# antoyang/TubeDETR

Measured on AMD Instinct MI355X. Metric: training clips/sec (fwd+bwd) at T=100 k=4 res=352, 1/2/4/8 MI355X, higher is better.
Workload: dtype bf16

## Files before the change

include/tubedetr_hip.h:

```cpp
#ifndef TUBEDETR_HIP_H
#define TUBEDETR_HIP_H
#include <stddef.h>
#include <stdint.h>
#ifdef __cplusplus
extern "C" {
#endif

#define TD_F32 0
#define TD_BF16 1
#define TD_U8 2
#define TD_OK 0
#define TD_ERR_INVALID (-1)
#define TD_ERR_LAUNCH (-2)

typedef void* td_stream_t;

const char* td_last_error(void);
int td_abi_version(void);

int td_set_deterministic(int on);
int td_get_deterministic(void);


#define TD_PROF_GEMM_128x128 0
#define TD_PROF_GEMM_128x64 1
#define TD_PROF_WGRAD 2
#define TD_PROF_GEMM_64x128 3
#define TD_PROF_PW_RESIDENT 4
#define TD_PROF_GEMM_256 5
#define TD_PROF_GEMM_256_PW 6
#define TD_PROF_FUSED 7
#define TD_PROF_CROSS_Q1 8
#define TD_PROF_WGRAD_SINGLE 9
#define TD_PROF_CHAIN 10
#define TD_PROF_FAMILIES 11
int td_prof_enable(int on);
int td_prof_collect(int family, int dtype, long long* launches, double* ms, double* flops);
int td_prof_collect_bytes(int family, int dtype, double* bytes);
int td_prof_dump(const char* path);
int td_debug_set_stamp_buffer(unsigned long long* buf);

typedef struct td_conv_desc {
  int N, Hs, Ws, C;
  int Ho, Wo;
  int R, S, stride, pad;
  int mode;
  int Nc;
  int ldc;
  int out_sp;
  int out_H, out_W;
  int aniso;
  int stride_w, pad_w;
} td_conv_desc;

typedef struct td_epilogue {
  const float* bias;
  const void* residual;
  const void* mask_src;
  int relu;
  int sigmoid;
  float dropout_p;
  uint32_t dropout_seed;
  float alpha;
  const uint32_t* dropout_counter;
} td_epilogue;

int td_conv_gemm(const void* src, const void* wmat, void* out, const td_conv_desc* d, const td_epilogue* e,
                 int dtype, td_stream_t stream);

typedef struct td_linear_ex_desc {
  int M, N, K1, K2;
  int lda1, lda2, ldc, ldr;
  int w_shared;
  long long rows1, rows2;
  const int* a1_map;
  const int* a2_map;
  const int* out_map;
  const int* res_map;
} td_linear_ex_desc;
int td_linear_ex(const void* a1, const void* a2, const void* wmat, void* out, const td_linear_ex_desc* x, const td_epilogue* e,
                 int dtype, td_stream_t stream);

int td_conv_wgrad(const void* g, const void* src, float* dw, const td_conv_desc* d, int ldg, int dtype, int splits,
                  td_stream_t stream);
int td_conv_wgrad_bias(const void* g, const void* src, float* dw, float* dbias, const td_conv_desc* d, int ldg, int dtype,
                       int splits, td_stream_t stream);

typedef struct td_wgrad_job {
  const void* g;
  const void* src;
  float* dW;
  const float* scale;
  td_conv_desc d;
  int ldg;
  int ci_real;
  float* dbias;
  int accumulate;
  int prezeroed;
} td_wgrad_job;
size_t td_conv_wgrad_batch_table_bytes(int n_jobs);
int td_conv_wgrad_batch(const td_wgrad_job* jobs, int n_jobs, int dtype, void* table_host, void* table_dev, size_t table_bytes,
                        td_stream_t stream);

typedef struct td_frame_source {
  const void* data;
  int dtype;
  int n;
  const int* index;
  const int* valid_hw;
} td_frame_source;
int td_frames_to_nhwc(const td_frame_source* srcs, int n_srcs, int C, int H, int W, int Cpad, const float* mean,
                      const float* inv_std, void* y, int dtype, td_stream_t stream);

size_t td_resnet_fwd_ws_bytes(int N, int H, int W, const int* nblocks, int dtype, int save);
int td_resnet_num_convs(const int* nblocks);
int td_resnet_fwd(const td_frame_source* srcs, int n_srcs, const float* mean, const float* inv_std, int N, int H, int W,
                  const int* nblocks, const void* const* w_fwd, const float* const* bias, int save, void* ws, size_t ws_bytes,
                  void** feat, int* feat_hw, int stem_pairs, int first_train_stage, int dtype, td_stream_t stream);
int td_bottleneck_fused(const void* x, void* out, const void* w1, const float* b1, const void* w2, const float* b2, const void* w3,
                        const float* b3, const void* wd, const float* bd, int N, int H, int W, int Cin, int dtype, td_stream_t stream);
int td_pw_chain2(const void* y2, const void* w3, const float* b3, const void* residual, void* out, const void* w1, const float* b1,
                 void* h1, int M, int planes, int dtype, td_stream_t stream);
int td_stem_pair_weights(const void* w_fwd_8, void* w_pairs, int Co, int dtype, td_stream_t stream);
int td_stem_pool(const void* x_pairs, const void* w_pairs, const float* bias, void* pooled, int N, int H, int W, int dtype,
                 td_stream_t stream);
size_t td_resnet_bwd_ws_bytes(int N, int H, int W, const int* nblocks, int first_train_stage, int dtype);
size_t td_resnet_bwd_table_bytes(const int* nblocks, int first_train_stage);
int td_resnet_bwd(const void* dfeat, int N, int N_fwd, int H, int W, const int* nblocks, int first_train_stage,
                  const void* const* w_dgrad, const float* const* scale, float* const* dW, const void* fwd_ws, void* ws,
                  size_t ws_bytes, void* table_host, void* table_dev, size_t table_bytes, int dW_prezeroed, int dtype, int only_stage, td_stream_t stream);

int td_weight_prep(const float* W, const float* bn_w, const float* bn_b, const float* bn_rm, const float* bn_rv,
                   const float* bias, int Co, int Ci, int R, int S, int Cpad, void* w_fwd, void* w_dgrad,
                   float* bias_out, float* scale_out, int dtype, td_stream_t stream);

typedef struct td_prep_item {
  const float* W;
  const float *bn_w, *bn_b, *bn_rm, *bn_rv, *bias;
  void *w_fwd, *w_dgrad;
  float *bias_out, *scale_out;
  int Co, Ci, RS, Cpad, Co_alloc, blk0;
} td_prep_item;
int td_weight_prep_batch(const td_prep_item* items_dev, int n, int total_blocks, int dtype, td_stream_t stream);

int td_wgrad_finalize(const float* dw_k, const float* scale, float* dW, int Co, int Ci, int R, int S, int Cpad,
                      int accumulate, td_stream_t stream);

int td_nchw_to_nhwc(const float* x, void* y, int N, int C, int H, int W, int Cpad, int dtype, td_stream_t stream);
int td_nhwc_to_nchw(const void* x, float* y, int N, int C, int H, int W, int dtype, td_stream_t stream);
int td_cast(const void* x, void* y, size_t n, int src_dtype, int dst_dtype, td_stream_t stream);

int td_maxpool3x3s2(const void* x, void* y, int N, int H, int W, int C, int dtype, td_stream_t stream);

int td_add_layernorm_fwd(const void* x, const void* r, const float* gamma, const float* beta, void* y, void* s_out,
                         float* mean, float* rstd, int rows, int cols, float eps, int dtype, td_stream_t stream);
int td_add_layernorm_bwd(const void* dy, const void* s, const float* mean, const float* rstd, const float* gamma,
                         const void* extra, void* ds, float* dgamma, float* dbeta, int rows, int cols, int dtype,
                         td_stream_t stream);

int td_colsum(const void* g, float* out, int rows, int cols, int ld, int dtype, td_stream_t stream);
int td_add(const void* a, const void* b, void* y, size_t n, int dtype, td_stream_t stream);

int td_relu_bwd(const void* dy, const void* y, void* g, size_t n, float scale, int dtype, td_stream_t stream);

int td_gelu_fwd(const void* x, void* y, size_t n, int dtype, td_stream_t stream);
int td_gelu_bwd(const void* dy, const void* x, void* dx, size_t n, int dtype, td_stream_t stream);

int td_dropout(const void* x, void* y, size_t n, float p, uint32_t seed, const uint32_t* dropout_counter, int dtype,
               td_stream_t stream);

int td_pos_sine(const uint8_t* mask, void* pos, int N, int h, int w, int npf, float temperature, int rows_per_image, int dtype,
                td_stream_t stream);

int td_rows_copy(const void* src, const int* src_map, const void* add, void* dst, const int* dst_map, int n_rows, int cols, int ld_src,
                 int ld_add, int ld_dst, int dtype, td_stream_t stream);
int td_rows_segment_sum(const void* in, const int* idx, const int* ptr, void* out, const int* out_map, int n_out, int cols, int ld_in,
                        int ld_out, int dtype, td_stream_t stream);

int td_mha_fwd(const void* q, const void* k, const void* v, const uint8_t* key_pad, void* out, float* probs,
               float* wavg, int B, int H, int Lq, int Lk, int hd, int ldq, int ldk, int ldv, int ldo, float scale,
               float dropout_p, uint32_t dropout_seed, const uint32_t* dropout_counter, int dtype, td_stream_t stream);
int td_mha_bwd(const void* q, const void* k, const void* v, const void* dout, const float* probs, const float* dwavg,
               void* dq, void* dk, void* dv, float* ds_ws, int B, int H, int Lq, int Lk, int hd, int ldq, int ldk,
               int ldv, int ldo, float scale, float dropout_p, uint32_t dropout_seed, const uint32_t* dropout_counter,
               int dtype, td_stream_t stream);

int td_cross_q1_fwd(const void* u, const void* mem, const void* pos, const uint8_t* key_pad, float* probs, float* wavg, void* zext,
                    int F, int S, int H, int E, int ldz, float dropout_p, uint32_t dropout_seed, const uint32_t* dropout_counter,
                    int dtype, td_stream_t stream);
int td_cross_q1_bwd(const void* u, const void* mem, const void* pos, const float* probs, const void* d_zext, const float* dwavg,
                    void* d_u, float* d_mem, int accumulate, int F, int S, int H, int E, int ldz, float dropout_p, uint32_t dropout_seed,
                    const uint32_t* dropout_counter, int dtype, td_stream_t stream);
int td_cross_q1_bwd_coef(const void* u, const void* mem, const void* pos, const float* probs, const void* d_zext, const float* dwavg,
                         void* d_u, void* coef, int coef_ld, int coef_col, int F, int S, int H, int E, int ldz, float dropout_p,
                         uint32_t dropout_seed, const uint32_t* dropout_counter, int dtype, td_stream_t stream);
int td_cross_q1_dmem(const void* coef, int coef_ld, const void* const* u, const void* const* d_zext, int n_layers, void* d_mem, int F, int S,
                     int H, int E, int ldz, int dtype, td_stream_t stream);
int td_head_blocks_expand(const float* W, const float* bias, float alpha, void* w_n, void* w_t, int E, int H, int dtype, td_stream_t stream);
int td_head_blocks_extract(const float* G, float alpha, float* dW, float* db, int E, int H, td_stream_t stream);

size_t td_mha_lean_stats_bytes(int B, int H, int Lq);
int td_mha_lean_fwd(const void* q, const void* k, const void* v, const uint8_t* key_pad, void* out, float* stats, int B, int H,
                    int Lq, int Lk, int hd, int ldq, int ldk, int ldv, int ldo, float scale, float dropout_p,
                    uint32_t dropout_seed, const uint32_t* dropout_counter, int dtype, td_stream_t stream);
int td_mha_lean_bwd(const void* q, const void* k, const void* v, const uint8_t* key_pad, const void* out, const void* dout,
                    float* stats, void* dq, void* dk, void* dv, int B, int H, int Lq, int Lk, int hd, int ldq, int ldk, int ldv,
                    int ldo, float scale, float dropout_p, uint32_t dropout_seed, const uint32_t* dropout_counter, int dtype,
                    td_stream_t stream);


#define TD_OPTIM_MAX_SEGMENTS 32
// ... 29 lines not shown
```

tubedetr_amd/_hip.py:

```python
from __future__ import annotations

import ctypes as C
import os

import torch

TD_F32, TD_BF16 = 0, 1
EXPECTED_ABI = 10
_LIB_PATH = os.environ.get("TD_HIP_LIB") or os.path.join(os.path.dirname(os.path.abspath(__file__)), "lib", "libtubedetr_hip.so")
_lib = None


class ConvDesc(C.Structure):
    _fields_ = [(n, C.c_int) for n in ("N", "Hs", "Ws", "C", "Ho", "Wo", "R", "S", "stride", "pad", "mode", "Nc", "ldc", "out_sp", "out_H", "out_W",
                                       "aniso", "stride_w", "pad_w")]


class PrepItem(C.Structure):
    _fields_ = [(n, C.c_void_p) for n in ("W", "bn_w", "bn_b", "bn_rm", "bn_rv", "bias", "w_fwd", "w_dgrad", "bias_out", "scale_out")] + \
               [(n, C.c_int) for n in ("Co", "Ci", "RS", "Cpad", "Co_alloc", "blk0")]


class WgradJob(C.Structure):
    _fields_ = [("g", C.c_void_p), ("src", C.c_void_p), ("dW", C.c_void_p), ("scale", C.c_void_p), ("d", ConvDesc), ("ldg", C.c_int), ("ci_real", C.c_int), ("dbias", C.c_void_p), ("accumulate", C.c_int), ("prezeroed", C.c_int)]


TD_U8 = 2


class FrameSource(C.Structure):
    _fields_ = [("data", C.c_void_p), ("dtype", C.c_int), ("n", C.c_int), ("index", C.c_void_p), ("valid_hw", C.c_void_p)]


class LinearExDesc(C.Structure):
    _fields_ = [(n, C.c_int) for n in ("M", "N", "K1", "K2", "lda1", "lda2", "ldc", "ldr", "w_shared")] + \
               [("rows1", C.c_longlong), ("rows2", C.c_longlong)] + [(n, C.c_void_p) for n in ("a1_map", "a2_map", "out_map", "res_map")]


class OptimSegment(C.Structure):
    _fields_ = [("begin", C.c_longlong), ("end", C.c_longlong), ("group", C.c_int), ("active", C.c_int)]


class Epilogue(C.Structure):
    _fields_ = [
        ("bias", C.c_void_p),
        ("residual", C.c_void_p),
        ("mask_src", C.c_void_p),
        ("relu", C.c_int),
        ("sigmoid", C.c_int),
        ("dropout_p", C.c_float),
        ("dropout_seed", C.c_uint32),
        ("alpha", C.c_float),
        ("dropout_counter", C.c_void_p),
    ]


_P, _I, _F, _U32, _SZ = C.c_void_p, C.c_int, C.c_float, C.c_uint32, C.c_size_t
_SIGS = {
    "td_prof_enable": [_I],
    "td_prof_dump": [C.c_char_p],
    "td_debug_set_stamp_buffer": [_P],
    "td_prof_collect": [_I, _I, C.POINTER(C.c_longlong), C.POINTER(C.c_double), C.POINTER(C.c_double)],
    "td_prof_collect_bytes": [_I, _I, C.POINTER(C.c_double)],
    "td_conv_gemm": [_P, _P, _P, C.POINTER(ConvDesc), C.POINTER(Epilogue), _I, _P],
    "td_conv_wgrad": [_P, _P, _P, C.POINTER(ConvDesc), _I, _I, _I, _P],
    "td_conv_wgrad_bias": [_P, _P, _P, _P, C.POINTER(ConvDesc), _I, _I, _I, _P],
    "td_conv_wgrad_batch": [C.POINTER(WgradJob), _I, _I, _P, _P, _SZ, _P],
    "td_resnet_num_convs": [C.POINTER(C.c_int)],
    "td_resnet_fwd": [C.POINTER(FrameSource), _I, C.POINTER(C.c_float), C.POINTER(C.c_float), _I, _I, _I, C.POINTER(C.c_int), C.POINTER(_P), C.POINTER(_P), _I, _P, _SZ,
                      C.POINTER(_P), C.POINTER(C.c_int), _I, _I, _I, _P],
    "td_bottleneck_fused": [_P, _P, _P, _P, _P, _P, _P, _P, _P, _P, _I, _I, _I, _I, _I, _P],
    "td_stem_pair_weights": [_P, _P, _I, _I, _P],
    "td_stem_pool": [_P, _P, _P, _P, _I, _I, _I, _I, _P],
    "td_pw_chain2": [_P, _P, _P, _P, _P, _P, _P, _P, _I, _I, _I, _P],
    "td_set_deterministic": [_I],
    "td_get_deterministic": [],
    "td_frames_to_nhwc": [C.POINTER(FrameSource), _I, _I, _I, _I, _I, C.POINTER(C.c_float), C.POINTER(C.c_float), _P, _I, _P],
    "td_resnet_bwd": [_P, _I, _I, _I, _I, C.POINTER(C.c_int), _I, C.POINTER(_P), C.POINTER(_P), C.POINTER(_P), _P, _P, _SZ, _P, _P, _SZ, _I, _I, _I, _P],
    "td_weight_prep_batch": [_P, _I, _I, _I, _P],
    "td_weight_prep": [_P, _P, _P, _P, _P, _P, _I, _I, _I, _I, _I, _P, _P, _P, _P, _I, _P],
    "td_wgrad_finalize": [_P, _P, _P, _I, _I, _I, _I, _I, _I, _P],
    "td_nchw_to_nhwc": [_P, _P, _I, _I, _I, _I, _I, _I, _P],
    "td_nhwc_to_nchw": [_P, _P, _I, _I, _I, _I, _I, _P],
    "td_cast": [_P, _P, _SZ, _I, _I, _P],
    "td_maxpool3x3s2": [_P, _P, _I, _I, _I, _I, _I, _P],
    "td_add_layernorm_fwd": [_P, _P, _P, _P, _P, _P, _P, _P, _I, _I, _F, _I, _P],
    "td_add_layernorm_bwd": [_P, _P, _P, _P, _P, _P, _P, _P, _P, _I, _I, _I, _P],
    "td_colsum": [_P, _P, _I, _I, _I, _I, _P],
    "td_add": [_P, _P, _P, _SZ, _I, _P],
    "td_relu_bwd": [_P, _P, _P, _SZ, _F, _I, _P],
    "td_gelu_fwd": [_P, _P, _SZ, _I, _P],
    "td_gelu_bwd": [_P, _P, _P, _SZ, _I, _P],
    "td_dropout": [_P, _P, _SZ, _F, _U32, _P, _I, _P],
    "td_pos_sine": [_P, _P, _I, _I, _I, _I, _F, _I, _I, _P],
    "td_linear_ex": [_P, _P, _P, _P, C.POINTER(LinearExDesc), C.POINTER(Epilogue), _I, _P],
    "td_rows_copy": [_P, _P, _P, _P, _P, _I, _I, _I, _I, _I, _I, _P],
    "td_rows_segment_sum": [_P, _P, _P, _P, _P, _I, _I, _I, _I, _I, _P],
    "td_criterion_fwd": [_P, _P, _P, _P, _P, _P, _P, _P, _P, _F, _F, _I, _I, _I, _I, _P, _P, _P, _P, _P, _P],
    "td_criterion_bwd": [_P, _P, _P, _P, _P, _P, _P, _P, _I, _I, _I, _P],
    "td_sted_decode": [_P, _P, _I, _I, _P],
    "td_grad_norm_clip": [_P, _SZ, C.POINTER(OptimSegment), _I, _F, _P, _SZ, _P, _P, _P],
    "td_adamw_ema_step": [_P, _P, _P, _P, _P, _SZ, C.POINTER(OptimSegment), _I, _P, _P, _P, _F, _F, _F, _F, _F, _P],
    "td_mha_fwd": [_P, _P, _P, _P, _P, _P, _P, _I, _I, _I, _I, _I, _I, _I, _I, _I, _F, _F, _U32, _P, _I, _P],
    "td_mha_bwd": [_P, _P, _P, _P, _P, _P, _P, _P, _P, _P, _I, _I, _I, _I, _I, _I, _I, _I, _I, _F, _F, _U32, _P, _I, _P],
    "td_cross_q1_fwd": [_P, _P, _P, _P, _P, _P, _P, _I, _I, _I, _I, _I, _F, _U32, _P, _I, _P],
    "td_cross_q1_bwd": [_P, _P, _P, _P, _P, _P, _P, _P, _I, _I, _I, _I, _I, _I, _F, _U32, _P, _I, _P],
    "td_cross_q1_bwd_coef": [_P, _P, _P, _P, _P, _P, _P, _P, _I, _I, _I, _I, _I, _I, _I, _F, _U32, _P, _I, _P],
    "td_cross_q1_dmem": [_P, _I, _P, _P, _I, _P, _I, _I, _I, _I, _I, _I, _P],
    "td_head_blocks_expand": [_P, _P, _F, _P, _P, _I, _I, _I, _P],
    "td_head_blocks_extract": [_P, _F, _P, _P, _I, _I, _P],
    "td_mha_lean_fwd": [_P, _P, _P, _P, _P, _P, _I, _I, _I, _I, _I, _I, _I, _I, _I, _F, _F, _U32, _P, _I, _P],
    "td_mha_lean_bwd": [_P, _P, _P, _P, _P, _P, _P, _P, _P, _P, _I, _I, _I, _I, _I, _I, _I, _I, _I, _F, _F, _U32, _P, _I, _P],
}
_SIZE_SIGS = {
    "td_grad_norm_ws_bytes": [],
    "td_mha_lean_stats_bytes": [_I, _I, _I],
    "td_conv_wgrad_batch_table_bytes": [_I],
    "td_resnet_bwd_table_bytes": [C.POINTER(C.c_int), _I],
    "td_resnet_fwd_ws_bytes": [_I, _I, _I, C.POINTER(C.c_int), _I, _I],
    "td_resnet_bwd_ws_bytes": [_I, _I, _I, C.POINTER(C.c_int), _I, _I],
}
EXPORTS = ["td_last_error", "td_abi_version"] + list(_SIGS) + list(_SIZE_SIGS)


def lib_path() -> str:
    return _LIB_PATH


def lib() -> C.CDLL:
    global _lib
    if _lib is None:
        if not os.path.exists(_LIB_PATH):
            raise RuntimeError(
                f"{_LIB_PATH} is missing: build it with `python -m tubedetr_amd.build` (or __graft_entry__.build()); "
                "tubedetr_amd has no CPU / eager fallback"
            )
        L = C.CDLL(_LIB_PATH)
        L.td_last_error.restype = C.c_char_p
        L.td_last_error.argtypes = []
        L.td_abi_version.restype = C.c_int
# ... 40 lines not shown
```

tubedetr_amd/csrc/api.cpp:

```cpp
#include <stdarg.h>

#include <atomic>
#include <mutex>
#include <vector>

#include "td_common.h"

namespace td {

static thread_local char g_err[512] = "";

void set_error(const char* fmt, ...) {
  va_list ap;
  va_start(ap, fmt);
  vsnprintf(g_err, sizeof(g_err), fmt, ap);
  va_end(ap);
}

int check_launch(const char* what) {
  hipError_t e = hipGetLastError();
  if (e != hipSuccess) {
    set_error("%s: launch failed: %s", what, hipGetErrorString(e));
    return TD_ERR_LAUNCH;
  }
// ... 49 lines not shown
}
extern "C" int td_get_deterministic(void) { return td::deterministic() ? 1 : 0; }

extern "C" int td_prof_enable(int on) {
  std::lock_guard<std::mutex> lk(td::g_prof_mu);
  td::g_prof.store(on != 0);
  if (on) {
    for (auto& r : td::g_recs) { td::g_pool.push_back(r.a); td::g_pool.push_back(r.b); }
    td::g_recs.clear();
  }
  return TD_OK;
}
extern "C" int td_prof_collect(int family, int dtype, long long* launches, double* ms, double* flops) {
  long long n = 0; double t = 0, f = 0;
  std::lock_guard<std::mutex> lk(td::g_prof_mu);
  for (auto& r : td::g_recs) {
    if (r.family != family || r.dtype != dtype) continue;
    if (hipEventSynchronize(r.b) != hipSuccess) { td::set_error("td_prof_collect: event sync failed"); return TD_ERR_LAUNCH; }
    float e = 0.f;
    hipEventElapsedTime(&e, r.a, r.b);
    n++; t += e; f += r.flops;
  }
  if (launches) *launches = n;
  if (ms) *ms = t;
  if (flops) *flops = f;
  return TD_OK;
}

extern "C" int td_prof_collect_bytes(int family, int dtype, double* bytes) {
  double b = 0;
  std::lock_guard<std::mutex> lk(td::g_prof_mu);
  for (auto& r : td::g_recs)
    if (r.family == family && r.dtype == dtype) b += r.bytes;
  if (bytes) *bytes = b;
  return TD_OK;
}

extern "C" int td_prof_dump(const char* path) {
  FILE* f = fopen(path, "w");
  if (!f) { td::set_error("td_prof_dump: cannot open %s", path); return TD_ERR_INVALID; }
  fprintf(f, "family,dtype,M,N,K,R,stride,mode,ms\n");
  std::lock_guard<std::mutex> lk(td::g_prof_mu);
  for (auto& r : td::g_recs) {
    hipEventSynchronize(r.b);
    float e = 0.f;
    hipEventElapsedTime(&e, r.a, r.b);
    fprintf(f, "%d,%d,%d,%d,%d,%d,%d,%d,%.5f\n", r.family, r.dtype, r.M, r.N, r.K, r.R, r.stride, r.mode, e);
  }
  fclose(f);
  return TD_OK;
}

extern "C" const char* td_last_error(void) { return td::g_err; }
extern "C" int td_abi_version(void) { return 10; }
```

tubedetr_amd/csrc/elementwise.hip:

```cpp
#include "td_common.h"

namespace td {

template <typename T>
__global__ void maxpool3x3s2_kernel(const T* x, T* y, int N, int H, int W, int C, int Ho, int Wo) {
  constexpr int VEC = 16 / sizeof(T);
  const int cv = C / VEC;
  const size_t n = (size_t)N * Ho * Wo * cv;
  const size_t idx = (size_t)blockIdx.x * blockDim.x + threadIdx.x;
  if (idx >= n) return;
  int c = (idx % cv) * VEC;
  size_t t = idx / cv;
  int wo = t % Wo; t /= Wo;
  int ho = t % Ho;
  int img = t / Ho;
  float m[VEC];
#pragma unroll
  for (int i = 0; i < VEC; ++i) m[i] = -INFINITY;
  for (int r = 0; r < 3; ++r) {
    int h = ho * 2 - 1 + r;
    if ((unsigned)h >= (unsigned)H) continue;
    for (int s = 0; s < 3; ++s) {
      int w = wo * 2 - 1 + s;
      if ((unsigned)w >= (unsigned)W) continue;
// ... 69 lines not shown
}
static bool aligned8(const void* a, const void* b, const void* c, const void* d) {
  return (((uintptr_t)a | (uintptr_t)b | (uintptr_t)c | (uintptr_t)d) & 7) == 0;
}

template <int NJ>
__global__ __launch_bounds__(256) void add_layernorm_fwd_v4_kernel(const u16* __restrict__ x, const u16* __restrict__ r, const float* __restrict__ gamma,
                                                                   const float* __restrict__ beta, u16* __restrict__ y, u16* __restrict__ s_out,
                                                                   float* __restrict__ mean, float* __restrict__ rstd, int rows, float eps) {
  constexpr int cols = NJ * 256;
  const int lane = threadIdx.x & 63;
  const int row = blockIdx.x * 4 + (threadIdx.x >> 6);
  if (row >= rows) return;
  const size_t base = (size_t)row * cols + lane * 4;
  float v[NJ][4];
  float sum = 0.f;
#pragma unroll
  for (int j = 0; j < NJ; ++j) {
    unpack4v(*(const uint2*)(x + base + 256 * j), v[j]);
    if (r) {
      float a[4];
      unpack4v(*(const uint2*)(r + base + 256 * j), a);
#pragma unroll
      for (int e = 0; e < 4; ++e) v[j][e] += a[e];
    }
#pragma unroll
    for (int e = 0; e < 4; ++e) sum += v[j][e];
  }
  const float mu = wave_sum(sum) * (1.f / cols);
  float var = 0.f;
#pragma unroll
  for (int j = 0; j < NJ; ++j)
#pragma unroll
    for (int e = 0; e < 4; ++e) {
      const float d = v[j][e] - mu;
      var += d * d;
    }
  var = wave_sum(var) * (1.f / cols);
  const float rs = rsqrtf(var + eps);
  if (lane == 0) {
    if (mean) mean[row] = mu;
    if (rstd) rstd[row] = rs;
  }
#pragma unroll
  for (int j = 0; j < NJ; ++j) {
    const float4 gm = *(const float4*)(gamma + lane * 4 + 256 * j), bt = *(const float4*)(beta + lane * 4 + 256 * j);
    if (s_out) *(uint2*)(s_out + base + 256 * j) = pack4_bf16(v[j]);
    float o[4] = {(v[j][0] - mu) * rs * gm.x + bt.x, (v[j][1] - mu) * rs * gm.y + bt.y, (v[j][2] - mu) * rs * gm.z + bt.z,
                  (v[j][3] - mu) * rs * gm.w + bt.w};
    *(uint2*)(y + base + 256 * j) = pack4_bf16(o);
  }
}

template <int NJ>
__global__ __launch_bounds__(256) void add_layernorm_bwd_v4_kernel(const u16* __restrict__ dy, const u16* __restrict__ s, const float* __restrict__ mean,
                                                                   const float* __restrict__ rstd, const float* __restrict__ gamma,
                                                                   const u16* __restrict__ extra, u16* __restrict__ ds, float* dgamma, float* dbeta,
                                                                   int rows) {
  constexpr int cols = NJ * 256;
  const int lane = threadIdx.x & 63;
  const int wid = blockIdx.x * 4 + (threadIdx.x >> 6);
  const int nw = gridDim.x * 4;
  float pg[NJ][4], pb[NJ][4], gm[NJ][4];
#pragma unroll
  for (int j = 0; j < NJ; ++j) {
    const float4 g4 = *(const float4*)(gamma + lane * 4 + 256 * j);
    gm[j][0] = g4.x; gm[j][1] = g4.y; gm[j][2] = g4.z; gm[j][3] = g4.w;
#pragma unroll
    for (int e = 0; e < 4; ++e) pg[j][e] = pb[j][e] = 0.f;
  }
  for (int row = wid; row < rows; row += nw) {
    const size_t base = (size_t)row * cols + lane * 4;
    const float mu = mean[row], rs = rstd[row];
    float xh[NJ][4], dg[NJ][4];
    float c1 = 0.f, c2 = 0.f;
#pragma unroll
    for (int j = 0; j < NJ; ++j) {
      float d[4], sv[4];
      unpack4v(*(const uint2*)(dy + base + 256 * j), d);
      unpack4v(*(const uint2*)(s + base + 256 * j), sv);
#pragma unroll
      for (int e = 0; e < 4; ++e) {
        xh[j][e] = (sv[e] - mu) * rs;
        dg[j][e] = d[e] * gm[j][e];
        c1 += dg[j][e];
        c2 += dg[j][e] * xh[j][e];
        pg[j][e] += d[e] * xh[j][e];
        pb[j][e] += d[e];
      }
    }
    c1 = wave_sum(c1) * (1.f / cols);
    c2 = wave_sum(c2) * (1.f / cols);
#pragma unroll
    for (int j = 0; j < NJ; ++j) {
      float o[4];
#pragma unroll
      for (int e = 0; e < 4; ++e) o[e] = rs * (dg[j][e] - c1 - xh[j][e] * c2);
      if (extra) {
        float ex[4];
        unpack4v(*(const uint2*)(extra + base + 256 * j), ex);
#pragma unroll
        for (int e = 0; e < 4; ++e) o[e] += ex[e];
      }
      *(uint2*)(ds + base + 256 * j) = pack4_bf16(o);
    }
  }
  __shared__ float redg[4][cols], redb[4][cols];
  const int wv = threadIdx.x >> 6;
#pragma unroll
  for (int j = 0; j < NJ; ++j)
#pragma unroll
    for (int e = 0; e < 4; ++e) {
      redg[wv][lane * 4 + 256 * j + e] = pg[j][e];
      redb[wv][lane * 4 + 256 * j + e] = pb[j][e];
    }
  __syncthreads();
  for (int c = threadIdx.x; c < cols; c += 256) {
    if (dgamma) atomicAdd(dgamma + c, redg[0][c] + redg[1][c] + redg[2][c] + redg[3][c]);
    if (dbeta) atomicAdd(dbeta + c, redb[0][c] + redb[1][c] + redb[2][c] + redb[3][c]);
  }
}

template <typename T>
__global__ __launch_bounds__(256) void add_layernorm_bwd_kernel(const T* dy, const T* s, const float* mean, const float* rstd,
                                                                const float* gamma, const T* extra, T* ds, float* dgamma,
                                                                float* dbeta, int rows, int cols) {
  const int lane = threadIdx.x & 63;
  const int wid = blockIdx.x * 4 + (threadIdx.x >> 6);
  const int nw = gridDim.x * 4;
  const int nj = (cols + 63) / 64;
  float pg[LN_MAXJ], pb[LN_MAXJ];
#pragma unroll
  for (int j = 0; j < LN_MAXJ; ++j) pg[j] = pb[j] = 0.f;
  for (int row = wid; row < rows; row += nw) {
    const size_t base = (size_t)row * cols;
    const float mu = mean[row], rs = rstd[row];
    float xh[LN_MAXJ], dg[LN_MAXJ];
    float c1 = 0.f, c2 = 0.f;
#pragma unroll
    for (int j = 0; j < LN_MAXJ; ++j) {
      xh[j] = dg[j] = 0.f;
      int c = lane + 64 * j;
      if (j < nj && c < cols) {
        float d = Elem<T>::load(dy, base + c);
        xh[j] = (Elem<T>::load(s, base + c) - mu) * rs;
        dg[j] = d * gamma[c];
        c1 += dg[j];
        c2 += dg[j] * xh[j];
        pg[j] += d * xh[j];
        pb[j] += d;
      }
    }
    c1 = wave_sum(c1) / cols;
    c2 = wave_sum(c2) / cols;
#pragma unroll
    for (int j = 0; j < LN_MAXJ; ++j) {
      int c = lane + 64 * j;
      if (j < nj && c < cols) {
        float o = rs * (dg[j] - c1 - xh[j] * c2);
        if (extra) o += Elem<T>::load(extra, base + c);
        Elem<T>::store(ds, base + c, o);
      }
    }
  }
  __shared__ float redg[4][64 * LN_MAXJ], redb[4][64 * LN_MAXJ];
  const int wv = threadIdx.x >> 6;
#pragma unroll
  for (int j = 0; j < LN_MAXJ; ++j) {
    if (j < nj) {
      redg[wv][lane + 64 * j] = pg[j];
      redb[wv][lane + 64 * j] = pb[j];
    }
  }
  __syncthreads();
  for (int c = threadIdx.x; c < cols; c += 256) {
    if (dgamma) atomicAdd(dgamma + c, redg[0][c] + redg[1][c] + redg[2][c] + redg[3][c]);
    if (dbeta) atomicAdd(dbeta + c, redb[0][c] + redb[1][c] + redb[2][c] + redb[3][c]);
  }
}

template <typename T>
__global__ void colsum_kernel(const T* g, float* out, int rows, int cols, int ld, int rows_per_block) {
  const int c = blockIdx.x * blockDim.x + threadIdx.x;
  if (c >= cols) return;
  const int r0 = blockIdx.y * rows_per_block;
  const int r1 = min(rows, r0 + rows_per_block);
  float acc = 0.f;
  for (int r = r0; r < r1; ++r) acc += Elem<T>::load(g, (size_t)r * ld + c);
  atomicAdd(out + c, acc);
}

template <typename T>
__global__ __launch_bounds__(256) void colsum_vec_kernel(const T* g, float* out, int rows, int cols, int ld, int rows_per_block) {
  constexpr int VEC = 16 / sizeof(T);
  __shared__ float red[8][32 * VEC + 1];
  const int cg = threadIdx.x & 31, rl = threadIdx.x >> 5;
  const int c0 = (blockIdx.x * 32 + cg) * VEC;
  const int r0 = blockIdx.y * rows_per_block;
  const int r1 = min(rows, r0 + rows_per_block);
  float acc[VEC];
#pragma unroll
  for (int i = 0; i < VEC; ++i) acc[i] = 0.f;
  if (c0 < cols) {
    for (int r = r0 + rl; r < r1; r += 8) {
      uint4 v = *(const uint4*)(g + (size_t)r * ld + c0);
      const T* e = (const T*)&v;
#pragma unroll
      for (int i = 0; i < VEC; ++i) acc[i] += Elem<T>::load(e, i);
    }
  }
#pragma unroll
  for (int i = 0; i < VEC; ++i) red[rl][cg * VEC + i] = acc[i];
  __syncthreads();
  for (int c = threadIdx.x; c < 32 * VEC; c += 256) {
// ... 192 lines not shown
  size_t n = (size_t)N * Ho * Wo * (C / vec);
  hipStream_t st = (hipStream_t)stream;
  TD_DISPATCH(dtype, (maxpool3x3s2_kernel<u16><<<nblk(n), 256, 0, st>>>((const u16*)x, (u16*)y, N, H, W, C, Ho, Wo)),
              (maxpool3x3s2_kernel<float><<<nblk(n), 256, 0, st>>>((const float*)x, (float*)y, N, H, W, C, Ho, Wo)),
              "td_maxpool3x3s2");
  return check_launch("td_maxpool3x3s2");
}

extern "C" int td_add_layernorm_fwd(const void* x, const void* r, const float* gamma, const float* beta, void* y,
                                    void* s_out, float* mean, float* rstd, int rows, int cols, float eps, int dtype,
                                    td_stream_t stream) {
  TD_REQUIRE(x && gamma && beta && y, "td_add_layernorm_fwd: null pointer");
  TD_REQUIRE(cols <= 64 * LN_MAXJ, "td_add_layernorm_fwd: cols > %d", 64 * LN_MAXJ);
  if (rows == 0) return TD_OK;
  hipStream_t st = (hipStream_t)stream;
  unsigned g = (rows + 3) / 4;
  if (dtype == TD_BF16 && (cols == 256 || cols == 768) && aligned8(x, r, y, s_out)) {
    if (cols == 256) add_layernorm_fwd_v4_kernel<1><<<g, 256, 0, st>>>((const u16*)x, (const u16*)r, gamma, beta, (u16*)y, (u16*)s_out, mean, rstd, rows, eps);
    else add_layernorm_fwd_v4_kernel<3><<<g, 256, 0, st>>>((const u16*)x, (const u16*)r, gamma, beta, (u16*)y, (u16*)s_out, mean, rstd, rows, eps);
    return check_launch("td_add_layernorm_fwd");
  }
  TD_DISPATCH(dtype,
              (add_layernorm_fwd_kernel<u16><<<g, 256, 0, st>>>((const u16*)x, (const u16*)r, gamma, beta, (u16*)y, (u16*)s_out, mean, rstd, rows, cols, eps)),
              (add_layernorm_fwd_kernel<float><<<g, 256, 0, st>>>((const float*)x, (const float*)r, gamma, beta, (float*)y, (float*)s_out, mean, rstd, rows, cols, eps)),
              "td_add_layernorm_fwd");
  return check_launch("td_add_layernorm_fwd");
}

extern "C" int td_add_layernorm_bwd(const void* dy, const void* s, const float* mean, const float* rstd,
                                    const float* gamma, const void* extra, void* ds, float* dgamma, float* dbeta,
                                    int rows, int cols, int dtype, td_stream_t stream) {
  TD_REQUIRE(dy && s && mean && rstd && gamma && ds, "td_add_layernorm_bwd: null pointer");
  TD_REQUIRE(cols <= 64 * LN_MAXJ, "td_add_layernorm_bwd: cols > %d", 64 * LN_MAXJ);
  if (rows == 0) return TD_OK;
  hipStream_t st = (hipStream_t)stream;
  unsigned g = (rows + 3) / 4;
  if (dtype == TD_BF16 && (cols == 256 || cols == 768) && aligned8(dy, s, ds, extra)) {
    unsigned gv = (rows + 31) / 32;
    if (gv > 1024) gv = 1024;
    if (deterministic()) gv = 1;
    if (cols == 256) add_layernorm_bwd_v4_kernel<1><<<gv, 256, 0, st>>>((const u16*)dy, (const u16*)s, mean, rstd, gamma, (const u16*)extra, (u16*)ds, dgamma, dbeta, rows);
    else add_layernorm_bwd_v4_kernel<3><<<gv, 256, 0, st>>>((const u16*)dy, (const u16*)s, mean, rstd, gamma, (const u16*)extra, (u16*)ds, dgamma, dbeta, rows);
    return check_launch("td_add_layernorm_bwd");
  }
  if (g > 256) g = 256;
  if (deterministic()) g = 1;
  TD_DISPATCH(dtype,
              (add_layernorm_bwd_kernel<u16><<<g, 256, 0, st>>>((const u16*)dy, (const u16*)s, mean, rstd, gamma, (const u16*)extra, (u16*)ds, dgamma, dbeta, rows, cols)),
              (add_layernorm_bwd_kernel<float><<<g, 256, 0, st>>>((const float*)dy, (const float*)s, mean, rstd, gamma, (const float*)extra, (float*)ds, dgamma, dbeta, rows, cols)),
              "td_add_layernorm_bwd");
  return check_launch("td_add_layernorm_bwd");
}

extern "C" int td_colsum(const void* g, float* out, int rows, int cols, int ld, int dtype, td_stream_t stream) {
  TD_REQUIRE(g && out, "td_colsum: null pointer");
  if (rows == 0 || cols == 0) return TD_OK;
  hipStream_t st = (hipStream_t)stream;
  const int vec = dtype == TD_BF16 ? 8 : 4;
  if (cols % vec == 0 && ld % vec == 0) {
    const int gx = (cols + 32 * vec - 1) / (32 * vec);
    int rpb = (int)(((long long)rows * gx + 511) / 512);
    if (rpb < 64) rpb = 64;
    if (deterministic()) rpb = rows;
    dim3 grid(gx, (rows + rpb - 1) / rpb);
    TD_DISPATCH(dtype, (colsum_vec_kernel<u16><<<grid, 256, 0, st>>>((const u16*)g, out, rows, cols, ld, rpb)),
                (colsum_vec_kernel<float><<<grid, 256, 0, st>>>((const float*)g, out, rows, cols, ld, rpb)), "td_colsum");
    return check_launch("td_colsum");
  }
  int rpb = (int)(((long long)rows * ((cols + 255) / 256) + 1023) / 1024);
  if (rpb < 8) rpb = 8;
  if (deterministic()) rpb = rows;
  dim3 grid((cols + 255) / 256, (rows + rpb - 1) / rpb);
  TD_DISPATCH(dtype, (colsum_kernel<u16><<<grid, 256, 0, st>>>((const u16*)g, out, rows, cols, ld, rpb)),
              (colsum_kernel<float><<<grid, 256, 0, st>>>((const float*)g, out, rows, cols, ld, rpb)), "td_colsum");
  return check_launch("td_colsum");
}

extern "C" int td_add(const void* a, const void* b, void* y, size_t n, int dtype, td_stream_t stream) {
  TD_REQUIRE(a && y, "td_add: null pointer");
  if (n == 0) return TD_OK;
  hipStream_t st = (hipStream_t)stream;
  unsigned g = nblk(n / 4 + 1);
  if (g > 4096) g = 4096;
  TD_REQUIRE(((uintptr_t)a | (uintptr_t)y | (uintptr_t)b) % 16 == 0, "td_add: pointers must be 16-byte aligned");
  TD_DISPATCH(dtype, (ew_kernel<u16, 0><<<g, 256, 0, st>>>((const u16*)a, (const u16*)b, (u16*)y, n, 1.f, 0, 0, nullptr)),
              (ew_kernel<float, 0><<<g, 256, 0, st>>>((const float*)a, (const float*)b, (float*)y, n, 1.f, 0, 0, nullptr)), "td_add");
  return check_launch("td_add");
}

extern "C" int td_relu_bwd(const void* dy, const void* y, void* g, size_t n, float scale, int dtype, td_stream_t stream) {
  TD_REQUIRE(dy && y && g, "td_relu_bwd: null pointer");
  if (n == 0) return TD_OK;
  hipStream_t st = (hipStream_t)stream;
  unsigned gr = nblk(n);
  if (gr > 4096) gr = 4096;
  TD_REQUIRE(((uintptr_t)dy | (uintptr_t)y | (uintptr_t)g) % 16 == 0, "td_relu_bwd: pointers must be 16-byte aligned");
  TD_DISPATCH(dtype, (ew_kernel<u16, 1><<<gr, 256, 0, st>>>((const u16*)dy, (const u16*)y, (u16*)g, n, scale, 0, 0, nullptr)),
              (ew_kernel<float, 1><<<gr, 256, 0, st>>>((const float*)dy, (const float*)y, (float*)g, n, scale, 0, 0, nullptr)), "td_relu_bwd");
  return check_launch("td_relu_bwd");
}

extern "C" int td_gelu_fwd(const void* x, void* y, size_t n, int dtype, td_stream_t stream) {
  TD_REQUIRE(x && y, "td_gelu_fwd: null pointer");
  if (n == 0) return TD_OK;
  hipStream_t st = (hipStream_t)stream;
  unsigned gr = nblk(n);
// ... 87 lines not shown
```

tubedetr_amd/csrc/gemm_conv.hip:

```cpp
#include <stdlib.h>

#include <type_traits>

#include "td_common.h"
#include <algorithm>
#include <vector>

#ifndef TD_WGRAD_EARLY_ISSUE
#define TD_WGRAD_EARLY_ISSUE 1
#endif
#ifndef TD_BIG_XCD_CONTIG
#define TD_BIG_XCD_CONTIG 1
#endif
namespace td {

struct GemmParams {
  const char* src;
  const char* w;
  char* out;
  td_conv_desc d;
  int M, K;
  uint32_t src_bytes, w_bytes;
  unsigned long long* dbg;
  const float* bias;
  const char* residual;
  const char* mask_src;
  int relu, sigmoid;
  float alpha;
  uint32_t drop_thresh;
  float drop_scale;
  uint32_t seed;
  const uint32_t* seed_dev;
  const char* src2;
  uint32_t src2_bytes;
  int K1, lda1, lda2, ldr;
  int w_shared;
  const int* a1_map;
  const int* a2_map;
  const int* out_map;
  const int* res_map;
  int tap_inner;
  int w_ld;
  int wtap[4];
  int use_wtap;
};

template <typename T>
struct Mfma;
template <>
struct Mfma<u16> {
  static __device__ __forceinline__ void run(const uint4& wf, const uint4& af, f32x4& acc) {
    acc = __builtin_amdgcn_mfma_f32_16x16x32_bf16(*(const bf16x8*)&wf, *(const bf16x8*)&af, acc, 0, 0, 0);
  }
};
template <>
struct Mfma<float> {
  static __device__ __forceinline__ void run(const uint4& wf, const uint4& af, f32x4& acc) {
    const float* a = (const float*)&wf;
    const float* b = (const float*)&af;
#pragma unroll
    for (int s = 0; s < 4; ++s) acc = __builtin_amdgcn_mfma_f32_16x16x4f32(a[s], b[s], acc, 0, 0, 0);
  }
};

template <typename T>
__device__ __forceinline__ void load4(const char* base, size_t off, float (&o)[4]);
template <>
__device__ __forceinline__ void load4<float>(const char* base, size_t off, float (&o)[4]) {
  float4 v = *(const float4*)(base + off * 4);
  o[0] = v.x; o[1] = v.y; o[2] = v.z; o[3] = v.w;
}
template <>
__device__ __forceinline__ void load4<u16>(const char* base, size_t off, float (&o)[4]) {
  uint2 v = *(const uint2*)(base + off * 2);
  o[0] = __uint_as_float(v.x << 16); o[1] = __uint_as_float(v.x & 0xffff0000u);
  o[2] = __uint_as_float(v.y << 16); o[3] = __uint_as_float(v.y & 0xffff0000u);
}
template <typename T, typename V>
__device__ __forceinline__ void unpack4(const V& v, float (&o)[4]);
template <>
__device__ __forceinline__ void unpack4<float, float4>(const float4& v, float (&o)[4]) {
  o[0] = v.x; o[1] = v.y; o[2] = v.z; o[3] = v.w;
}
template <>
__device__ __forceinline__ void unpack4<u16, uint2>(const uint2& v, float (&o)[4]) {
  o[0] = __uint_as_float(v.x << 16); o[1] = __uint_as_float(v.x & 0xffff0000u);
  o[2] = __uint_as_float(v.y << 16); o[3] = __uint_as_float(v.y & 0xffff0000u);
}
typedef __bf16 bf16x2_t __attribute__((ext_vector_type(2)));
__device__ __forceinline__ uint32_t pack_bf16x2(float lo, float hi) {
  bf16x2_t v = {(__bf16)lo, (__bf16)hi};
  return *(uint32_t*)&v;
}
template <typename T>
__device__ __forceinline__ void unpack16(const uint4& v, float (&o)[16 / sizeof(T)]);
template <>
__device__ __forceinline__ void unpack16<float>(const uint4& v, float (&o)[4]) {
  o[0] = __uint_as_float(v.x); o[1] = __uint_as_float(v.y); o[2] = __uint_as_float(v.z); o[3] = __uint_as_float(v.w);
}
template <>
__device__ __forceinline__ void unpack16<u16>(const uint4& v, float (&o)[8]) {
  o[0] = __uint_as_float(v.x << 16); o[1] = __uint_as_float(v.x & 0xffff0000u);
  o[2] = __uint_as_float(v.y << 16); o[3] = __uint_as_float(v.y & 0xffff0000u);
  o[4] = __uint_as_float(v.z << 16); o[5] = __uint_as_float(v.z & 0xffff0000u);
  o[6] = __uint_as_float(v.w << 16); o[7] = __uint_as_float(v.w & 0xffff0000u);
}
template <typename T>
__device__ __forceinline__ uint4 pack16(const float (&v)[16 / sizeof(T)]);
template <>
__device__ __forceinline__ uint4 pack16<float>(const float (&v)[4]) {
  return make_uint4(__float_as_uint(v[0]), __float_as_uint(v[1]), __float_as_uint(v[2]), __float_as_uint(v[3]));
}
template <>
__device__ __forceinline__ uint4 pack16<u16>(const float (&v)[8]) {
  return make_uint4(pack_bf16x2(v[0], v[1]), pack_bf16x2(v[2], v[3]), pack_bf16x2(v[4], v[5]), pack_bf16x2(v[6], v[7]));
}
template <typename T>
__device__ __forceinline__ void store4(char* base, size_t off, const float (&v)[4]);
template <>
__device__ __forceinline__ void store4<float>(char* base, size_t off, const float (&v)[4]) {
  *(float4*)(base + off * 4) = make_float4(v[0], v[1], v[2], v[3]);
}
template <>
__device__ __forceinline__ void store4<u16>(char* base, size_t off, const float (&v)[4]) {
  uint2 o;
  o.x = (uint32_t)f32_to_bf16(v[0]) | ((uint32_t)f32_to_bf16(v[1]) << 16);
  o.y = (uint32_t)f32_to_bf16(v[2]) | ((uint32_t)f32_to_bf16(v[3]) << 16);
  *(uint2*)(base + off * 2) = o;
}

__device__ __forceinline__ float sigmoidf_(float x) { return 1.f / (1.f + __expf(-x)); }

typedef __attribute__((address_space(3))) void* lds_ptr_t;

#ifndef TD_NT
#define TD_NT 3
#endif
typedef uint32_t u32x4_t __attribute__((ext_vector_type(4)));
typedef uint32_t u32x2_t __attribute__((ext_vector_type(2)));
__device__ __forceinline__ uint4 ld16(const char* p) {
#if TD_NT & 1
  const u32x4_t v = __builtin_nontemporal_load((const u32x4_t*)p);
  return make_uint4(v.x, v.y, v.z, v.w);
#else
  return *(const uint4*)p;
#endif
// ... 272 lines not shown
  issue_tile(nxt);                                                                  \
  if ((j) >= 0) compute_tile(cur);
    for (int it = -2; it < nk; it += 3) {
      TD_CG_STEP(smem1, smem0, it)
      if (it + 1 >= nk) break;
      TD_CG_STEP(smem2, smem1, it + 1)
      if (it + 2 >= nk) break;
      TD_CG_STEP(smem0, smem2, it + 2)
    }
#undef TD_CG_STEP
    asm volatile("s_waitcnt vmcnt(0)" ::: "memory");
    TD_STAMP(2);
    fetch_epilogue_operands();
  }

  asm volatile("s_waitcnt lgkmcnt(0)" ::: "memory");
  __builtin_amdgcn_s_barrier();
  TD_STAMP(3);
  float* stg = (float*)((wave < 2 ? smem0 : smem1) + (wave & 1) * (WM * WN * 4));
  const float alpha = p.alpha;
#pragma unroll
  for (int j = 0; j < TM; ++j) {
    const int row = j * 16 + lr;
#pragma unroll
    for (int i = 0; i < TN; ++i) {
      const int c = (i * 4 + lg) ^ (row & (CPRW - 1));
      f32x4 a = acc[i][j];
      *(float4*)(stg + row * WN + c * 4) = make_float4(a[0] * alpha, a[1] * alpha, a[2] * alpha, a[3] * alpha);
    }
  }
  asm volatile("s_waitcnt lgkmcnt(0)" ::: "memory");
  float bias[EPL];
#pragma unroll
  for (int r = 0; r < EPL; ++r) bias[r] = (p.bias && n + r < d.Nc) ? p.bias[n + r] : 0.f;
  TD_STAMP(4);
  const uint32_t eff_seed = effective_seed(p.seed, p.drop_thresh ? p.seed_dev : nullptr);
#pragma unroll
  for (int it = 0; it < NIT; ++it) {
    if (!live[it]) continue;
    const int row = it * RPI + rsub;
    const int sw = row & (CPRW - 1);
    float v[EPL];
#pragma unroll
    for (int q = 0; q < EPL / 4; ++q) {
      float4 f = *(const float4*)(stg + row * WN + (((cc * (EPL / 4) + q) ^ sw) * 4));
      v[4 * q + 0] = f.x + bias[4 * q + 0]; v[4 * q + 1] = f.y + bias[4 * q + 1];
      v[4 * q + 2] = f.z + bias[4 * q + 2]; v[4 * q + 3] = f.w + bias[4 * q + 3];
    }
    const size_t off = offs[it];
    if (vec_ok) {
      if (p.residual) {
        float r8[EPL];
        unpack16<T>(res[it], r8);
#pragma unroll
        for (int r = 0; r < EPL; ++r) v[r] += r8[r];
      }
      if (p.relu) {
#pragma unroll
        for (int r = 0; r < EPL; ++r) v[r] = fmaxf(v[r], 0.f);
      }
      if (p.sigmoid) {
#pragma unroll
        for (int r = 0; r < EPL; ++r) v[r] = sigmoidf_(v[r]);
      }
      if (p.mask_src) {
        float m8[EPL];
        unpack16<T>(msk[it], m8);
#pragma unroll
        for (int r = 0; r < EPL; ++r) v[r] = m8[r] > 0.f ? v[r] : 0.f;
      }
      if (p.drop_thresh) {
#pragma unroll
        for (int r = 0; r < EPL; ++r) v[r] = dropout_keep(eff_seed, (uint32_t)(off + r), p.drop_thresh) ? v[r] * p.drop_scale : 0.f;
      }
      st16(p.out + off * ES, pack16<T>(v));
    } else {
      const int cnt = min(EPL, d.Nc - n);
      for (int r = 0; r < cnt; ++r) {
        float x = v[r];
        if (p.residual) x += Elem<T>::load(p.residual, (GX ? roffs[it] : off) + r);
        if (p.relu) x = fmaxf(x, 0.f);
        if (p.sigmoid) x = sigmoidf_(x);
        if (p.mask_src) x = Elem<T>::load(p.mask_src, off + r) > 0.f ? x : 0.f;
        if (p.drop_thresh) x = dropout_keep(eff_seed, (uint32_t)(off + r), p.drop_thresh) ? x * p.drop_scale : 0.f;
        Elem<T>::store(p.out, off + r, x);
      }
    }
  }
  TD_STAMP(5);
#undef TD_STAMP
}

#ifndef TD_ABL
#define TD_ABL 0
#endif
template <int OFF>
__device__ __forceinline__ u32x4_t lds_read16(uint32_t addr) {
  u32x4_t r;
#if TD_ABL & 4
  asm volatile("" : "=v"(r) : "v"(addr));
#else
  asm volatile("ds_read_b128 %0, %1 offset:%2" : "=v"(r) : "v"(addr), "n"(OFF));
#endif
  return r;
}
template <int N>
__device__ __forceinline__ void wait_vmcnt() {
  asm volatile("s_waitcnt vmcnt(%0)" ::"n"(N) : "memory");
}
template <int I>
using ic = std::integral_constant<int, I>;

#ifndef TD_BIG8_AUX_W
#define TD_BIG8_AUX_W 0
#endif
#ifndef TD_BIG8_AUX_X
#define TD_BIG8_AUX_X 0
#endif
template <bool TU, bool RES>
__global__ __launch_bounds__(512, 1) void conv_gemm_big8_kernel(GemmParams p) {
  using T = u16;
  constexpr int ES = 2, BM = 256, BN = 256, BK = 64, NW = 8, VEC = 8;
  constexpr int WM = 128, WN = 64, TM = 8, TN = 4;
  constexpr int STAGE = (BM + BN) * 128, WREG = BM * 128;
  constexpr uint32_t OOB = 0xFFFFFFF0u;
  constexpr int MAXT = 160;
  constexpr int STG = 16 * WN * ES;
  __shared__ __attribute__((aligned(16))) char smem[2 * STAGE];
  __shared__ __attribute__((aligned(16))) uint4 ktab[MAXT];
  __shared__ __attribute__((aligned(16))) char stg_all[NW * STG];

  const td_conv_desc& d = p.d;
  const int t = threadIdx.x;
// ... 201 lines not shown
      for (int j = 0; j < TM; ++j) acc[i][j] = f32x4{0.f, 0.f, 0.f, 0.f};
    taddr = tab0 + 2 * 16;
    f32x4 bs[TN];
#pragma unroll
    for (int i = 0; i < TN; ++i) bs[i] = p.bias ? *(const f32x4*)(p.bias + n0 + wx * WN + i * 16 + lg * 4) : f32x4{0.f, 0.f, 0.f, 0.f};
    wait_vmcnt<7>();
    __builtin_amdgcn_s_barrier();
    if (wy == 1) __builtin_amdgcn_s_barrier();
    TD_STAMP(1);
    const int npair = (nk + 1) / 2;
#pragma unroll 1
    for (int it = 0; it < npair; ++it) {
      phase(ic<0>{}, ic<0>{}); phase(ic<0>{}, ic<1>{}); phase(ic<0>{}, ic<2>{}); phase(ic<0>{}, ic<3>{});
      phase(ic<1>{}, ic<0>{}); phase(ic<1>{}, ic<1>{}); phase(ic<1>{}, ic<2>{}); phase(ic<1>{}, ic<3>{});
    }
    if (wy == 0) __builtin_amdgcn_s_barrier();
    TD_STAMP(2);
    asm volatile("s_waitcnt vmcnt(0) lgkmcnt(0)" ::: "memory");
    asm volatile("s_nop 15\n\ts_nop 15" ::: "memory");
#pragma unroll
    for (int i = 0; i < TN; ++i)
#pragma unroll
      for (int j = 0; j < TM; ++j) asm volatile("" : "+v"(acc[i][j]));
#pragma unroll
    for (int i = 0; i < TN; ++i) asm volatile("" : "+v"(bs[i]));
    const int vb_next = vb + (int)gridDim.x;
    const bool more = tile_ok(vb_next);
    if (more) {
      tile_addr(tile_m0(vb_next), tile_n0(vb_next));
      prologue_issue();
    }
    TD_STAMP(3);
    uint4 mk[2][2];
    auto seg_off = [&](int j, int h) -> uint32_t {
      const int m = m0 + wy * WM + j * 16 + h * 8 + rsub;
      return m < p.M ? ((uint32_t)m * (uint32_t)d.ldc + (uint32_t)(n0 + wx * WN + cc * 8)) * ES : OOB;
    };
    auto fetch_mask = [&](int j, int b) {
#pragma unroll
      for (int h = 0; h < 2; ++h) {
        const uint32_t off = seg_off(j, h);
        mk[b][h] = off != OOB ? ld16(p.mask_src + off) : make_uint4(0, 0, 0, 0);
      }
    };
    auto put = [&](int j) {
#pragma unroll
      for (int i = 0; i < TN; ++i) {
        const f32x4 a = acc[i][j];
        float v[4] = {a[0] * alpha + bs[i][0], a[1] * alpha + bs[i][1], a[2] * alpha + bs[i][2], a[3] * alpha + bs[i][3]};
        if constexpr (RES) {
          const int m = m0 + wy * WM + j * 16 + lr;
          if (m < p.M) {
            const uint2 rr = *(const uint2*)(p.residual + ((size_t)m * d.ldc + n0 + wx * WN + i * 16 + lg * 4) * ES);
            v[0] += __uint_as_float(rr.x << 16); v[1] += __uint_as_float(rr.x & 0xffff0000u);
            v[2] += __uint_as_float(rr.y << 16); v[3] += __uint_as_float(rr.y & 0xffff0000u);
          }
        }
        if (p.relu) {
#pragma unroll
          for (int r = 0; r < 4; ++r) v[r] = fmaxf(v[r], 0.f);
        }
        const uint32_t lo = pack_bf16x2(v[0], v[1]), hi = pack_bf16x2(v[2], v[3]);
        asm volatile("ds_write_b64 %0, %1" ::"v"(swa[i]), "v"(u32x2_t{lo, hi}) : "memory");
      }
    };
    if (p.mask_src) fetch_mask(0, 0);
    put(0);
    u32x4_t o0, o1;
    asm volatile("ds_read_b128 %0, %1" : "=v"(o0) : "v"(sra) : "memory");
    asm volatile("ds_read_b128 %0, %1 offset:1024" : "=v"(o1) : "v"(sra) : "memory");
#pragma unroll
    for (int j = 0; j < TM; ++j) {
      const int b = j & 1;
      if (j + 1 < TM) {
        if (p.mask_src) fetch_mask(j + 1, b ^ 1);
        put(j + 1);
        asm volatile("s_waitcnt lgkmcnt(4)" : "+v"(o0), "+v"(o1) : : "memory");
      } else {
        asm volatile("s_waitcnt lgkmcnt(0)" : "+v"(o0), "+v"(o1) : : "memory");
      }
      u32x4_t s0 = o0, s1 = o1;
      if (j + 1 < TM) {
        asm volatile("ds_read_b128 %0, %1" : "=v"(o0) : "v"(sra) : "memory");
        asm volatile("ds_read_b128 %0, %1 offset:1024" : "=v"(o1) : "v"(sra) : "memory");
      }
      if (p.mask_src) {
        float x8[8], m8[8];
        unpack16<T>(make_uint4(s0.x, s0.y, s0.z, s0.w), x8);
        unpack16<T>(mk[b][0], m8);
#pragma unroll
        for (int r = 0; r < 8; ++r) x8[r] = m8[r] > 0.f ? x8[r] : 0.f;
        const uint4 q0 = pack16<T>(x8);
        s0 = u32x4_t{q0.x, q0.y, q0.z, q0.w};
        unpack16<T>(make_uint4(s1.x, s1.y, s1.z, s1.w), x8);
        unpack16<T>(mk[b][1], m8);
#pragma unroll
        for (int r = 0; r < 8; ++r) x8[r] = m8[r] > 0.f ? x8[r] : 0.f;
        const uint4 q1 = pack16<T>(x8);
        s1 = u32x4_t{q1.x, q1.y, q1.z, q1.w};
      }
      __builtin_amdgcn_raw_buffer_store_b128(s0, rs_out, (int)seg_off(j, 0), 0, 0);
      __builtin_amdgcn_raw_buffer_store_b128(s1, rs_out, (int)seg_off(j, 1), 0, 0);
    }
    TD_STAMP(5);
    if (p.dbg && t == 0) p.dbg[(size_t)vb * 8 + 7] = wall_clock64();
    if (!more) break;
// ... 191 lines not shown
  if (grp == 1) __builtin_amdgcn_s_barrier();
  TD_STAMP(1);
  const int ntri = (nk + 2) / 3;
#pragma unroll 1
  for (int it = 0; it < ntri; ++it) {
    phase(ic<0>{}, ic<0>{}); phase(ic<0>{}, ic<1>{});
    phase(ic<1>{}, ic<0>{}); phase(ic<1>{}, ic<1>{});
    phase(ic<2>{}, ic<0>{}); phase(ic<2>{}, ic<1>{});
  }
  if (grp == 0) __builtin_amdgcn_s_barrier();
  TD_STAMP(2);
  asm volatile("s_waitcnt vmcnt(0) lgkmcnt(0)" ::: "memory");
  asm volatile("s_nop 15\n\ts_nop 15" ::: "memory");
#pragma unroll
  for (int i = 0; i < TN; ++i)
#pragma unroll
    for (int j = 0; j < TM; ++j) asm volatile("" : "+v"(acc[i][j]));
  fetch_chunk(0, 0);
  __builtin_amdgcn_s_barrier();
  TD_STAMP(3);
  float* stg = (float*)(smem + wave * (CR * WN * 4));
  const float alpha = p.alpha;
  float bias[EPL];
#pragma unroll
  for (int r = 0; r < EPL; ++r) bias[r] = p.bias ? p.bias[n + r] : 0.f;
#pragma unroll
  for (int c = 0; c < NCH; ++c) {
    const int b = c & 1;
    {
      const int row = lr;
#pragma unroll
      for (int i = 0; i < TN; ++i) {
        const int cx = (i * 4 + lg) ^ (row & (CPRW - 1));
        const f32x4 a = acc[i][c];
        *(float4*)(stg + row * WN + cx * 4) = make_float4(a[0] * alpha, a[1] * alpha, a[2] * alpha, a[3] * alpha);
      }
    }
    if (c + 1 < NCH) fetch_chunk(c + 1, b ^ 1);
    asm volatile("s_waitcnt lgkmcnt(0)" ::: "memory");
#pragma unroll
    for (int it = 0; it < NIT; ++it) {
      const int row = it * RPI + rsub;
      const int sw = row & (CPRW - 1);
      float v[EPL];
#pragma unroll
      for (int q = 0; q < EPL / 4; ++q) {
        const float4 f = *(const float4*)(stg + row * WN + (((cc * (EPL / 4) + q) ^ sw) * 4));
        v[4 * q + 0] = f.x + bias[4 * q + 0]; v[4 * q + 1] = f.y + bias[4 * q + 1];
        v[4 * q + 2] = f.z + bias[4 * q + 2]; v[4 * q + 3] = f.w + bias[4 * q + 3];
      }
      if (p.residual) {
        float r8[EPL];
        unpack16<T>(res[b][it], r8);
#pragma unroll
        for (int r = 0; r < EPL; ++r) v[r] += r8[r];
      }
      if (p.relu) {
#pragma unroll
        for (int r = 0; r < EPL; ++r) v[r] = fmaxf(v[r], 0.f);
      }
      if (p.mask_src) {
        float m8[EPL];
        unpack16<T>(msk[b][it], m8);
#pragma unroll
        for (int r = 0; r < EPL; ++r) v[r] = m8[r] > 0.f ? v[r] : 0.f;
      }
      if (live[b][it]) st16(p.out + offs[b][it] * ES, pack16<T>(v));
    }
    asm volatile("s_waitcnt lgkmcnt(0)" ::: "memory");
  }
  TD_STAMP(5);
#undef TD_STAMP
}

template <int NKT, bool RES, bool MSK>
__global__ __launch_bounds__(256, 2) void pw_resident2_kernel(GemmParams p, int MT, int P) {
  using T = u16;
  constexpr int ES = 2;
  constexpr uint32_t OOB = 0xFFFFFFF0u;
  constexpr int WM = 32, WN = 64, TM = 2, TN = 4;
  constexpr int CPRW = WN / 4, EPL = 8, LPR = WN / EPL, RPI = 64 / LPR, NIT = WM / RPI;
  constexpr int NOPS = NIT * ((RES ? 1 : 0) + (MSK ? 1 : 0));
  constexpr bool AHEAD = NOPS > 0 && !(RES && MSK && NKT == 4);
  constexpr int NA = 2 * NKT;
  constexpr int AUX_NT = (TD_NT & 2) ? 2 : 0;
  __shared__ __attribute__((aligned(16))) char sA0[32768];
  __shared__ __attribute__((aligned(16))) char sA1[32768];
  __shared__ __attribute__((aligned(16))) char sT[4 * 16 * WN * 4];
  const td_conv_desc& d = p.d;
  const int t = threadIdx.x;
  const int wave = __builtin_amdgcn_readfirstlane(t >> 6), lane = t & 63;
  const int NT = d.Nc >> 7;
  const int xcd = blockIdx.x & 7, local = blockIdx.x >> 3;
  const int GPX = P / NT;
  const int nt = local % NT, gl = local / NT;
  if (gl >= GPX) return;
  const int gid = xcd * GPX + gl, G = 8 * GPX;
  const int lrow = lane >> 3, chunk = (lane & 7) ^ lrow;
  const uint32_t out_bytes = (uint32_t)p.M * (uint32_t)d.ldc * ES;
  const __amdgpu_buffer_rsrc_t rs_src = __builtin_amdgcn_make_buffer_rsrc((void*)p.src, 0, p.src_bytes, 0x00020000);
  const __amdgpu_buffer_rsrc_t rs_out = __builtin_amdgcn_make_buffer_rsrc((void*)p.out, 0, out_bytes, 0x00020000);
  const __amdgpu_buffer_rsrc_t rs_res = __builtin_amdgcn_make_buffer_rsrc((void*)(RES ? p.residual : p.out), 0, out_bytes, 0x00020000);
  const __amdgpu_buffer_rsrc_t rs_msk = __builtin_amdgcn_make_buffer_rsrc((void*)(MSK ? p.mask_src : p.out), 0, out_bytes, 0x00020000);
  const int n0 = nt * 128;
  const int HoWo = d.Ho * d.Wo;
  const bool strided = d.stride != 1;
// ... 61 lines not shown
    for (int i = 0; i < TN; ++i)
#pragma unroll
      for (int j = 0; j < TM; ++j) acc[i][j] = f32x4{0.f, 0.f, 0.f, 0.f};
#pragma unroll
    for (int kt = 0; kt < NKT; ++kt)
#pragma unroll
      for (int ks = 0; ks < 2; ++ks) {
        const int cidx = ks * 4 + lg;
        uint4 af[TM];
#pragma unroll
        for (int j = 0; j < TM; ++j) {
          const int row = wy * WM + j * 16 + lr;
          af[j] = *(const uint4*)(cur + kt * 8192 + row * 128 + ((cidx ^ (row & 7)) << 4));
        }
#pragma unroll
        for (int i = 0; i < TN; ++i)
#pragma unroll
          for (int j = 0; j < TM; ++j) Mfma<T>::run(wfr[kt][ks][i], af[j], acc[i][j]);
      }
    asm volatile("s_waitcnt lgkmcnt(0)" ::: "memory");
    __builtin_amdgcn_s_barrier();
    issue_A(cur, mt + 2 * G);
    if constexpr (AHEAD) fetch_ops(mt + G, B ^ 1);
    if constexpr (NOPS > 0) {
      wait_vmcnt<NA + (AHEAD ? NOPS : 0)>();
      __builtin_amdgcn_sched_barrier(0);
    }
    constexpr int RB = AHEAD ? B : 0;
#pragma unroll
    for (int j = 0; j < TM; ++j) {
#pragma unroll
      for (int i = 0; i < TN; ++i) {
        const int c = (i * 4 + lg) ^ (lr & (CPRW - 1));
        const f32x4 a = acc[i][j];
        *(float4*)(stg + lr * WN + c * 4) = make_float4(a[0], a[1], a[2], a[3]);
      }
      asm volatile("s_waitcnt lgkmcnt(0)" ::: "memory");
#pragma unroll
      for (int h = 0; h < 16 / RPI; ++h) {
        const int it = j * (16 / RPI) + h;
        const int row = h * RPI + rsub;
        const int sw = row & (CPRW - 1);
        float v[EPL];
#pragma unroll
        for (int q = 0; q < EPL / 4; ++q) {
          const float4 f = *(const float4*)(stg + row * WN + (((cc * (EPL / 4) + q) ^ sw) * 4));
          v[4 * q + 0] = f.x + bias[4 * q + 0]; v[4 * q + 1] = f.y + bias[4 * q + 1];
          v[4 * q + 2] = f.z + bias[4 * q + 2]; v[4 * q + 3] = f.w + bias[4 * q + 3];
        }
        const uint32_t off = seg_off(mt, it);
        if constexpr (RES) {
          float r8[EPL];
          unpack16<T>(make_uint4(res[RB][it].x, res[RB][it].y, res[RB][it].z, res[RB][it].w), r8);
#pragma unroll
          for (int r = 0; r < EPL; ++r) v[r] += r8[r];
        }
        if (p.relu) {
#pragma unroll
          for (int r = 0; r < EPL; ++r) v[r] = fmaxf(v[r], 0.f);
        }
        if constexpr (MSK) {
          float m8[EPL];
          unpack16<T>(make_uint4(msk[RB][it].x, msk[RB][it].y, msk[RB][it].z, msk[RB][it].w), m8);
#pragma unroll
          for (int r = 0; r < EPL; ++r) v[r] = m8[r] > 0.f ? v[r] : 0.f;
        }
        if (p.drop_thresh) {
#pragma unroll
          for (int r = 0; r < EPL; ++r) v[r] = dropout_keep(drop_seed, off / ES + (uint32_t)r, p.drop_thresh) ? v[r] * p.drop_scale : 0.f;
        }
        const uint4 o = pack16<T>(v);
        __builtin_amdgcn_raw_buffer_store_b128(u32x4_t{o.x, o.y, o.z, o.w}, rs_out, (int)off, 0, AUX_NT);
      }
      asm volatile("s_waitcnt lgkmcnt(0)" ::: "memory");
    }
  };

  int mt = gid;
  issue_A(sA0, mt);
  issue_A(sA1, mt + G);
  if constexpr (AHEAD) fetch_ops(mt, 0);
  while (mt < MT) {
    step(sA0, sA1, mt, ic<0>{});
    mt += G;
    if (mt >= MT) break;
    step(sA1, sA0, mt, ic<1>{});
    mt += G;
  }
  asm volatile("s_waitcnt vmcnt(0)" ::: "memory");
}

struct WgradParams {
  const char* g;
  const char* src;
  float* dw;
  const float* scale;
  float* dbias;
  td_conv_desc d;
  int M, K, ldg, mper;
  uint32_t g_bytes, src_bytes;
  int out_mode;
  int ci_real;
  int tn, tk, first;
  int cls;
  unsigned long long* stamps;
};
// ... 800 lines not shown
      }
      sub.w_bytes = wbytes - (size_t)(wp - (const char*)w_dgrad);
      const int rc = conv_gemm_launch(g, wp, (char*)dx + ooff, &c, &ec, dtype, stream, &sub);
      if (rc) return rc;
    }
  return TD_OK;
}

extern "C" int td_conv_gemm(const void* src, const void* wmat, void* out, const td_conv_desc* d, const td_epilogue* e,
                            int dtype, td_stream_t stream) {
  TD_REQUIRE(src && wmat && out && d, "td_conv_gemm: null pointer");
  static const int parity = [] { const char* e_ = getenv("TD_DGRAD_S2_PARITY"); return e_ ? atoi(e_) : 1; }();
  if (parity && dtype == TD_BF16 && d->mode == 1 && d->stride == 2 && d->R == 3 && d->S == 3 && d->pad == 1 && !d->aniso && d->out_sp <= 1 &&
      d->Ho == 2 * d->Hs && d->Wo == 2 * d->Ws && d->C % 64 == 0 && d->ldc >= d->Nc && !(e && (e->dropout_p > 0.f || e->sigmoid))) {
    int rc = validate(d, dtype, "td_conv_gemm");
    if (rc) return rc;
    return conv_dgrad_s2_by_parity(src, wmat, out, d, e, dtype, stream);
  }
  return conv_gemm_launch(src, wmat, out, d, e, dtype, stream, nullptr);
}

static int conv_gemm_launch(const void* src, const void* wmat, void* out, const td_conv_desc* d, const td_epilogue* e, int dtype,
                            td_stream_t stream, const WeightSubset* sub) {
  TD_REQUIRE(src && wmat && out && d, "td_conv_gemm: null pointer");
  int rc = validate(d, dtype, "td_conv_gemm");
  if (rc) return rc;
  GemmParams p;
  memset(&p, 0, sizeof(p));
  p.src = (const char*)src;
  p.w = (const char*)wmat;
  p.out = (char*)out;
  p.d = *d;
  if (p.d.out_sp < 1) p.d.out_sp = 1;
  p.M = d->N * d->Ho * d->Wo;
  p.K = d->R * d->S * d->C;
  {
    const double es = dtype == TD_BF16 ? 2.0 : 4.0;
    const double sb = (double)d->N * d->Hs * d->Ws * d->C * es, wb = (double)d->Nc * p.K * es;
    TD_REQUIRE(sb < 4294967000.0 && wb < 4294967000.0, "td_conv_gemm: operand exceeds the 4 GiB buffer-descriptor range");
    p.src_bytes = (uint32_t)sb;
    p.w_bytes = (uint32_t)wb;
  }
  if (sub) {
    p.w_ld = sub->w_ld;
    p.w_bytes = (uint32_t)sub->w_bytes;
    p.use_wtap = sub->ntap > 1;
    for (int i = 0; i < 4; ++i) p.wtap[i] = sub->wtap[i];
  }
  p.alpha = 1.f;
  p.dbg = g_dbg;
  if (e) {
    p.bias = e->bias;
    p.residual = (const char*)e->residual;
    p.mask_src = (const char*)e->mask_src;
    p.relu = e->relu;
    p.sigmoid = e->sigmoid;
    if (e->alpha != 0.f) p.alpha = e->alpha;
    if (e->dropout_p > 0.f) {
      TD_REQUIRE(e->dropout_p < 1.f, "td_conv_gemm: dropout_p must be < 1");
      p.drop_thresh = (uint32_t)((double)e->dropout_p * 4294967296.0);
      if (p.drop_thresh == 0) p.drop_thresh = 1;
      p.drop_scale = 1.f / (1.f - e->dropout_p);
      p.seed = e->dropout_seed;
      p.seed_dev = e->dropout_counter;
    }
  }
  TD_REQUIRE(d->ldc >= d->Nc, "td_conv_gemm: ldc < Nc");
  hipStream_t st = (hipStream_t)stream;
  static const int n_cu = [] {
    int dev = 0, cus = 256;
    if (hipGetDevice(&dev) == hipSuccess) (void)hipDeviceGetAttribute(&cus, hipDeviceAttributeMultiprocessorCount, dev);
    return cus;
  }();
  {
    static const int persist = [] { const char* e_ = getenv("TD_PW_PERSIST"); return e_ ? atoi(e_) : 1; }();
    static const int persist_dropout = [] { const char* e_ = getenv("TD_PW_PERSIST_DROPOUT"); return e_ ? atoi(e_) : 1; }();
    const bool pw0 = d->R == 1 && d->S == 1 && d->pad == 0 && p.d.out_sp == 1 && !d->aniso &&
                     ((d->stride == 1 && d->Hs == d->Ho && d->Ws == d->Wo) ||
                      (d->stride > 1 && d->mode == 0 && (d->Ho - 1) * d->stride < d->Hs && (d->Wo - 1) * d->stride < d->Ws));
    const int NTp = d->Nc / 128, Pp = 2 * n_cu / 8;
    const bool shape_ok = pw0 && !p.w_ld && dtype == TD_BF16 && p.K % 64 == 0 && p.K <= 256 && d->Nc % 128 == 0 &&
                          (NTp == 1 || NTp == 2 || NTp == 4 || NTp == 8 || NTp == 16) && Pp >= NTp && d->ldc % 8 == 0 && !p.sigmoid &&
                          p.alpha == 1.f && n_cu % 8 == 0 && (!p.drop_thresh || persist_dropout) && (double)p.M * d->ldc < 2147483000.0;
    const int MTp = cdiv(p.M, 64);
    const int groups = shape_ok ? 8 * (Pp / NTp) : 1;
    if (persist && shape_ok && MTp >= persist_min_tiles() * groups && !(persist == 2 && p.mask_src) && !(persist == 3 && d->mode != 0)) {
      const bool prof_ = prof_on();
      if (prof_) {
        prof_begin(TD_PROF_PW_RESIDENT, dtype, 2.0 * p.M * d->Nc * p.K, st, p.M, d->Nc, p.K, d->R, d->stride, d->mode);
        const double es_ = 2.0;
        double by = ((double)p.M * p.K + (double)d->Nc * p.K + (double)p.M * d->Nc) * es_;
        if (p.residual) by += (double)p.M * d->Nc * es_;
        if (p.mask_src) by += (double)p.M * d->Nc * es_;
        prof_set_bytes(by);
      }
      const int nkt = p.K / 64;
      const bool hr = p.residual != nullptr, hm = p.mask_src != nullptr;
      dim3 g2(2 * n_cu);
#define TD_PWR(NK)                                                                               \
  do {                                                                                           \
    if (hr && hm) pw_resident2_kernel<NK, true, true><<<g2, 256, 0, st>>>(p, MTp, Pp);          \
    else if (hr) pw_resident2_kernel<NK, true, false><<<g2, 256, 0, st>>>(p, MTp, Pp);          \
    else if (hm) pw_resident2_kernel<NK, false, true><<<g2, 256, 0, st>>>(p, MTp, Pp);          \
    else pw_resident2_kernel<NK, false, false><<<g2, 256, 0, st>>>(p, MTp, Pp);                 \
  } while (0)
      if (nkt == 1) TD_PWR(1);
// ... 81 lines not shown
    else TD_LAUNCH(float, 128, 128);
  }
#undef TD_LAUNCH
  if (prof) prof_end(st);
  return check_launch("td_conv_gemm");
}

extern "C" int td_linear_ex(const void* a1, const void* a2, const void* wmat, void* out, const td_linear_ex_desc* x, const td_epilogue* e,
                            int dtype, td_stream_t stream) {
  TD_REQUIRE(a1 && wmat && out && x, "td_linear_ex: null pointer");
  TD_REQUIRE(dtype == TD_F32 || dtype == TD_BF16, "td_linear_ex: bad dtype %d", dtype);
  const int vec = dtype == TD_BF16 ? 8 : 4, bk = dtype == TD_BF16 ? 64 : 32;
  const int es = dtype == TD_BF16 ? 2 : 4;
  const int K2 = a2 ? x->K2 : 0;
  TD_REQUIRE(x->M >= 1 && x->N >= 1 && x->K1 >= vec && K2 >= 0, "td_linear_ex: bad sizes");
  TD_REQUIRE(x->K1 % vec == 0 && K2 % vec == 0 && x->lda1 % vec == 0 && (!a2 || x->lda2 % vec == 0), "td_linear_ex: K1 / K2 / lda must be multiples of %d", vec);
  TD_REQUIRE(!a2 || x->K1 % bk == 0, "td_linear_ex: with a second source K1=%d must be a multiple of the K tile (%d)", x->K1, bk);
  TD_REQUIRE(x->lda1 >= x->K1 && (!a2 || x->lda2 >= K2) && x->ldc >= x->N, "td_linear_ex: row stride smaller than the row");
  TD_REQUIRE(x->rows1 >= 1 && (!a2 || x->rows2 >= 1) && (x->a1_map || x->rows1 >= x->M) && (!a2 || x->a2_map || x->rows2 >= x->M),
             "td_linear_ex: source has fewer rows than M and no row map");
  GemmParams p;
  memset(&p, 0, sizeof(p));
  p.src = (const char*)a1;
  p.src2 = (const char*)a2;
  p.w = (const char*)wmat;
  p.out = (char*)out;
  p.M = x->M;
  p.K = x->K1 + K2;
  p.K1 = x->K1;
  p.lda1 = x->lda1;
  p.lda2 = a2 ? x->lda2 : 0;
  p.ldr = x->ldr > 0 ? x->ldr : x->ldc;
  p.w_shared = (a2 && x->w_shared) ? 1 : 0;
  TD_REQUIRE(!p.w_shared || K2 == x->K1, "td_linear_ex: a shared weight needs K2 == K1");
  p.a1_map = x->a1_map;
  p.a2_map = a2 ? x->a2_map : nullptr;
  p.out_map = x->out_map;
  p.res_map = x->res_map;
  td_conv_desc d;
  memset(&d, 0, sizeof(d));
  d.N = 1; d.Hs = x->M; d.Ws = 1; d.C = p.K; d.Ho = x->M; d.Wo = 1; d.R = d.S = 1; d.stride = 1; d.Nc = x->N; d.ldc = x->ldc; d.out_sp = 1;
  p.d = d;
  {
    const double b1 = (double)x->rows1 * x->lda1 * es, b2 = a2 ? (double)x->rows2 * x->lda2 * es : 16.0, wb = (double)x->N * (p.w_shared ? x->K1 : p.K) * es;
    TD_REQUIRE(b1 < 4294967000.0 && b2 < 4294967000.0 && wb < 4294967000.0, "td_linear_ex: operand exceeds the 4 GiB buffer-descriptor range");
    p.src_bytes = (uint32_t)b1;
    p.src2_bytes = (uint32_t)b2;
    p.w_bytes = (uint32_t)wb;
  }
  p.alpha = 1.f;
  if (e) {
    p.bias = e->bias;
    p.residual = (const char*)e->residual;
    p.mask_src = (const char*)e->mask_src;
    p.relu = e->relu;
    p.sigmoid = e->sigmoid;
    if (e->alpha != 0.f) p.alpha = e->alpha;
    if (e->dropout_p > 0.f) {
      TD_REQUIRE(e->dropout_p < 1.f, "td_linear_ex: dropout_p must be < 1");
      p.drop_thresh = (uint32_t)((double)e->dropout_p * 4294967296.0);
      if (p.drop_thresh == 0) p.drop_thresh = 1;
      p.drop_scale = 1.f / (1.f - e->dropout_p);
      p.seed = e->dropout_seed;
      p.seed_dev = e->dropout_counter;
    }
  }
  hipStream_t st = (hipStream_t)stream;
  const bool narrow = x->N <= 64;
  const int tiles128 = cdiv(p.M, 128) * cdiv(x->N, 128);
  const bool small_m = !narrow && (tiles128 < 512 || p.K <= 512);
  const int BMsel = small_m ? 64 : 128, BNsel = narrow ? 64 : 128;
  dim3 grid(8 * cdiv(cdiv(p.M, BMsel), 8) * cdiv(x->N, BNsel));
  const bool prof = prof_on();
  if (prof) {
    prof_begin(narrow ? TD_PROF_GEMM_128x64 : (small_m ? TD_PROF_GEMM_64x128 : TD_PROF_GEMM_128x128), dtype, 2.0 * p.M * x->N * p.K, st, p.M, x->N, p.K, 1, 1, 2);
    double by = ((double)p.M * p.K + (double)x->N * p.K + (double)p.M * x->N) * es;
    if (p.residual) by += (double)p.M * x->N * es;
    if (p.mask_src) by += (double)p.M * x->N * es;
    prof_set_bytes(by);
  }
#define TD_LX(TT)                                                                                     \
  do {                                                                                                \
    if (narrow) conv_gemm_kernel<TT, 128, 64, 2, true, false, true><<<grid, 256, 0, st>>>(p);         \
    else if (small_m) conv_gemm_kernel<TT, 64, 128, 2, true, false, true><<<grid, 256, 0, st>>>(p);   \
    else conv_gemm_kernel<TT, 128, 128, 2, true, false, true><<<grid, 256, 0, st>>>(p);               \
  } while (0)
  if (dtype == TD_BF16) TD_LX(u16);
  else TD_LX(float);
#undef TD_LX
  if (prof) prof_end(st);
  return check_launch("td_linear_ex");
}

static int wgrad_stages() {
  static const int nstg = [] { const char* e = getenv("TD_WGRAD_STAGES"); return (e && atoi(e) == 2) ? 2 : 4; }();
  return nstg;
}

static int wgrad_fill(WgradParams& p, const void* g, const void* src, const td_conv_desc* d, int ldg, int dtype, int* splits_io,
                      int auto_mode, const char* who) {
  int rc = validate(d, dtype, who);
  if (rc) return rc;
  const int vec = dtype == TD_BF16 ? 8 : 4;
  TD_REQUIRE(d->mode == 0 && !d->aniso, "%s: isotropic forward geometry expected", who);
  TD_REQUIRE(d->Nc % vec == 0 && ldg % vec == 0, "%s: Nc=%d / ldg=%d must be multiples of %d", who, d->Nc, ldg, vec);
  memset(&p, 0, sizeof(p));
// ... 240 lines not shown
```

tubedetr_amd/functional.py:

```python
from __future__ import annotations

import math
from typing import Optional

import torch
from torch.autograd import Function

from . import ops

Tensor = torch.Tensor

_EPOCH = [0]


def invalidate_prepared():
    _EPOCH[0] += 1


class _PrepEntry:
    __slots__ = ("base_ref", "offset", "shape", "bn", "dtype", "need_dgrad", "cpad", "co_alloc", "res", "ver", "dims")


class _PrepRegistry:

# ... 159 lines not shown
        if not q.requires_grad:
            continue
        if _USES.get(id(q), 0) != 1 or q.grad is not None or q._backward_hooks or getattr(q, "_post_accumulate_grad_hooks", None):
            return False
    return True


def _flush_deferred_wgrads():
    with _DEFER_LOCK:
        jobs = list(_DEFER_JOBS)
        _DEFER_JOBS.clear()
        _USES.clear()
        _ARMED[0] = False
    if jobs:
        ops.linear_wgrad_batch(jobs)


def _drop_stale_deferred():
    if _ARMED[0]:
        with _DEFER_LOCK:
            _DEFER_JOBS.clear()
            _USES.clear()
            _ARMED[0] = False


def _arm():
    with _DEFER_LOCK:
        if _ARMED[0]:
            return
        _ARMED[0] = True
    torch.autograd.Variable._execution_engine.queue_callback(_flush_deferred_wgrads)


def _wgrad(g: Tensor, x: Tensor, defer: bool, *, want_bias: bool, out: Optional[Tensor] = None, dbias: Optional[Tensor] = None,
           x2: Optional[Tensor] = None):
    M, K = x.shape
    N = g.shape[1]
    dev = g.device
    if not defer:
        db = dbias if dbias is not None else (ops.zeros_f32(N, dev) if want_bias else None)
        dW = ops.linear_wgrad(g, x, out=out, dbias=db)
        if x2 is not None:
            ops.linear_wgrad(g, x2, out=dW)
        return dW, db
    dW = out if out is not None else torch.empty((N, K), dtype=torch.float32, device=dev)
    db = dbias if dbias is not None else (torch.empty(N, dtype=torch.float32, device=dev) if want_bias else None)
    with _DEFER_LOCK:
        _DEFER_JOBS.append((g, x, dW.data_ptr(), db.data_ptr() if db is not None else None))
        if x2 is not None:
            _DEFER_JOBS.append((g, x2, dW.data_ptr(), None, True))
    return dW, db


class LinearFn(Function):

    @staticmethod
    def forward(ctx, x, W, b, relu: bool, dropout_p: float, seed: int):
        _note_use(ctx.needs_input_grad[1], W, b)
        N = W.shape[0]
        vec = ops.vec_of(x.dtype)
        Np = ops.pad_to(N, vec)
        wf, wd, _, _ = prepared(W, x.dtype, pad_out=Np if Np != N else 0)
        bias = b.detach() if b is not None else None
        if bias is not None and Np != N:
            bias = torch.cat([bias, bias.new_zeros(Np - N)])
        y = ops.linear_fwd(x, wf, bias, relu=relu, dropout_p=dropout_p, seed=seed)
        ctx.save_for_backward(x, y if (relu or dropout_p > 0) else None, wd)
        ctx.cfg = (relu, dropout_p, seed, N, Np, b is not None)
        ctx.params = (W, b)
        return y[:, :N].contiguous() if Np != N else y

    @staticmethod
    def backward(ctx, dy):
        _arm()
        x, y, wd = ctx.saved_tensors
        relu, p, seed, N, Np, has_b = ctx.cfg
        dy = dy.contiguous()
        if Np != N:
            g = dy.new_zeros((dy.shape[0], Np))
            g[:, :N] = dy
            dy = g
        if relu:
            g = ops.relu_bwd(dy, y, 1.0 / (1.0 - p) if p > 0 else 1.0)
        elif p > 0:
            g = ops.dropout(dy, p, seed)
        else:
            g = dy
        dx = ops.linear_fwd(g, wd) if ctx.needs_input_grad[0] else None
        want_w, want_b = ctx.needs_input_grad[1], has_b and ctx.needs_input_grad[2]
        dW = db = None
        if want_w:
            dW_full, db_full = _wgrad(g, x, _can_defer(*ctx.params), want_bias=want_b)
            dW = dW_full[:N]
            db = db_full[:N] if want_b else None
        elif want_b:
            db = ops.colsum(g)[:N]
        return dx, dW, db, None, None, None


def linear(x, W, b=None, relu=False, dropout_p=0.0, training=False):
    p = dropout_p if training else 0.0
    return LinearFn.apply(x, W, b, relu, p, _seed() if p > 0 else 0)


class FFNFn(Function):

    @staticmethod
    def forward(ctx, x, W1, b1, W2, b2, p: float, seed1: int, seed2: int):
        _note_use(ctx.needs_input_grad[1], W1, b1, W2, b2)
        w1f, w1d, _, _ = prepared(W1, x.dtype)
        w2f, w2d, _, _ = prepared(W2, x.dtype)
        h = ops.linear_fwd(x, w1f, b1.detach(), relu=True, dropout_p=p, seed=seed1)
        y = ops.linear_fwd(h, w2f, b2.detach(), dropout_p=p, seed=seed2)
        ctx.save_for_backward(x, h, w1d, w2d)
        ctx.cfg = (p, seed1, seed2)
        ctx.params = (W1, b1, W2, b2)
        return y

    @staticmethod
    def backward(ctx, dy):
        _arm()
        x, h, w1d, w2d = ctx.saved_tensors
        p, seed1, seed2 = ctx.cfg
        defer = _can_defer(*ctx.params)
        g2 = ops.dropout(dy.contiguous(), p, seed2) if p > 0 else dy.contiguous()
        dW2, db2 = _wgrad(g2, h, defer, want_bias=True)
        dh = ops.linear_fwd(g2, w2d, mask_src=h, alpha=1.0 / (1.0 - p) if p > 0 else 1.0)
        dW1, db1 = _wgrad(dh, x, defer, want_bias=True)
        dx = ops.linear_fwd(dh, w1d) if ctx.needs_input_grad[0] else None
        return dx, dW1, db1, dW2, db2, None, None, None


def ffn(x, W1, b1, W2, b2, dropout_p=0.0, training=False):
    p = dropout_p if training else 0.0
    return FFNFn.apply(x, W1, b1, W2, b2, p, _seed() if p > 0 else 0, _seed() if p > 0 else 0)


class AddLayerNormFn(Function):

    @staticmethod
    def forward(ctx, x, r, gamma, beta, eps: float):
        y, s, mean, rstd = ops.add_layernorm_fwd(x, r, gamma.detach(), beta.detach(), eps)
        ctx.save_for_backward(s, mean, rstd, gamma.detach())
        ctx.has_r = r is not None
        return y

    @staticmethod
    def backward(ctx, dy):
        s, mean, rstd, gamma = ctx.saved_tensors
        ds, dg, db = ops.add_layernorm_bwd(dy.contiguous(), s, mean, rstd, gamma)
        return ds, (ds if ctx.has_r else None), dg, db, None


def add_layernorm(x, r, gamma, beta, eps=1e-5):
    return AddLayerNormFn.apply(x, r, gamma, beta, eps)


class AddFn(Function):

    @staticmethod
    def forward(ctx, a, b):
        return ops.add(a, b)

    @staticmethod
    def backward(ctx, g):
        return g, g


class MHAFn(Function):

    @staticmethod
    def forward(ctx, q_in, q_pos, k_in, v_in, W_in, b_in, W_out, b_out, key_pad, B, Lq, Lk, H, need_w, p_attn, seed_attn, p_out, seed_out):
        _note_use(ctx.needs_input_grad[4], W_in, b_in, W_out, b_out)
        E = q_in.shape[1]
        dt = q_in.dtype
        same_qk = k_in is None
        bi = b_in.detach()

        def proj(x_, w_, b_):
            return ops.linear_ex(x_, w_, b_, a2=q_pos, w_shared=True) if q_pos is not None else ops.linear_fwd(x_, w_, b_)

        if same_qk:
            wqk_f, wqk_d, _, _ = prepared(W_in[: 2 * E], dt)
            qk = proj(q_in, wqk_f, bi[: 2 * E]).view(B, Lq, 2 * E)
            q, k = qk[..., :E], qk[..., E:]
            wd_list = (wqk_d,)
        else:
            wq_f, wq_d, _, _ = prepared(W_in[:E], dt)
            wk_f, wk_d, _, _ = prepared(W_in[E : 2 * E], dt)
            q = proj(q_in, wq_f, bi[:E]).view(B, Lq, E)
            k = ops.linear_fwd(k_in, wk_f, bi[E : 2 * E]).view(B, Lk, E)
            wd_list = (wq_d, wk_d)
        wv_f, wv_d, _, _ = prepared(W_in[2 * E :], dt)
        v = ops.linear_fwd(v_in, wv_f, bi[2 * E :]).view(B, Lk, E)
        scale = 1.0 / math.sqrt(E // H)
        lean = not need_w and ops.mha_lean_ok(q, k, v, H)
        if lean:
            ctxv, probs, kp = ops.mha_lean_fwd(q, k, v, key_pad, H, scale, dropout_p=p_attn, seed=seed_attn)
            wavg = None
        else:
            ctxv, probs, wavg = ops.mha_fwd(q, k, v, key_pad, H, scale, need_wavg=need_w, dropout_p=p_attn, seed=seed_attn)
            kp = None
        wo_f, wo_d, _, _ = prepared(W_out, dt)
        out = ops.linear_fwd(ctxv.view(B * Lq, E), wo_f, b_out.detach(), dropout_p=p_out, seed=seed_out)
        ctx.save_for_backward(q_in, q_pos, k_in, v_in, q, k, v, probs, ctxv, wv_d, wo_d, *wd_list)
        ctx.lean, ctx.kp = lean, kp
        ctx.cfg = (B, Lq, Lk, H, E, same_qk, scale, p_attn, seed_attn, p_out, seed_out)
        ctx.params = (W_in, b_in, W_out, b_out)
        return out, (wavg if need_w else None)

    @staticmethod
    def backward(ctx, dout, dwavg):
        _arm()
        q_in, q_pos, k_in, v_in, q, k, v, probs, ctxv, wv_d, wo_d, *wd_list = ctx.saved_tensors
        B, Lq, Lk, H, E, same_qk, scale, p_attn, seed_attn, p_out, seed_out = ctx.cfg
        dt = q_in.dtype
        dev = q_in.device
        defer = _can_defer(*ctx.params)
        g = ops.dropout(dout.contiguous(), p_out, seed_out) if p_out > 0 else dout.contiguous()
        if defer:
            dW_in = torch.empty((3 * E, E), dtype=torch.float32, device=dev)
            db_in = torch.empty(3 * E, dtype=torch.float32, device=dev)
        else:
            dW_in = ops.zeros_f32((3 * E, E), dev)
            db_in = ops.zeros_f32(3 * E, dev)
        dW_out, db_out = _wgrad(g, ctxv.view(B * Lq, E), defer, want_bias=True)
        dctx = ops.linear_fwd(g, wo_d).view(B, Lq, E)
        if same_qk:
            dqk = torch.empty((B, Lq, 2 * E), dtype=dt, device=dev)
            dq, dk = dqk[..., :E], dqk[..., E:]
        else:
            dq = torch.empty((B, Lq, E), dtype=dt, device=dev)
            dk = torch.empty((B, Lk, E), dtype=dt, device=dev)
        dv = torch.empty((B, Lk, E), dtype=dt, device=dev)
        dwa = dwavg.contiguous().float() if dwavg is not None else None
        if ctx.lean:
            ops.mha_lean_bwd(q, k, v, ctx.kp, ctxv, dctx, probs, H, scale, dq, dk, dv, dropout_p=p_attn, seed=seed_attn)
        else:
            ops.mha_bwd(q, k, v, dctx, probs, dwa, H, scale, dq, dk, dv, dropout_p=p_attn, seed=seed_attn)
        dv2 = dv.view(B * Lk, E)
        _wgrad(dv2, v_in, defer, want_bias=True, out=dW_in[2 * E :], dbias=db_in[2 * E :])
        d_v_in = ops.linear_fwd(dv2, wv_d) if ctx.needs_input_grad[3] else None
        d_q_in = d_k_in = None
        need_q = ctx.needs_input_grad[0] or (q_pos is not None and ctx.needs_input_grad[1])
        if same_qk:
            dqk2 = dqk.view(B * Lq, 2 * E)
            _wgrad(dqk2, q_in, defer, want_bias=True, out=dW_in[: 2 * E], dbias=db_in[: 2 * E], x2=q_pos)
            if need_q:
                d_q_in = ops.linear_fwd(dqk2, wd_list[0])
        else:
            dq2, dk2 = dq.view(B * Lq, E), dk.view(B * Lk, E)
            _wgrad(dq2, q_in, defer, want_bias=True, out=dW_in[:E], dbias=db_in[:E], x2=q_pos)
            _wgrad(dk2, k_in, defer, want_bias=True, out=dW_in[E : 2 * E], dbias=db_in[E : 2 * E])
            if need_q:
                d_q_in = ops.linear_fwd(dq2, wd_list[0])
            if ctx.needs_input_grad[2]:
                d_k_in = ops.linear_fwd(dk2, wd_list[1])
        return (d_q_in if ctx.needs_input_grad[0] else None, d_q_in if (q_pos is not None and ctx.needs_input_grad[1]) else None, d_k_in, d_v_in,
                dW_in, db_in, dW_out, db_out) + (None,) * 10


class _CrossKVShared:

    def __init__(self, mem, pos, n_layers, E):
        self.mem, self.pos, self.n_layers, self.E = mem, pos, n_layers, E
        self.dK = self.dV = None
        self.written = set()
        self.wk_d = self.wv_d = None

    def grads(self, like):
        if self.dK is None:
            self.dK = torch.empty((self.mem.shape[0], self.n_layers * self.E), dtype=like.dtype, device=like.device)
            self.dV = torch.empty_like(self.dK)
        return self.dK, self.dV


class CrossKVFn(Function):

    @staticmethod
    def forward(ctx, mem, pos, shared, *w_and_b):
        E, dt = shared.E, mem.dtype
        Ws, bs = w_and_b[0::2], w_and_b[1::2]
        kf, vf, kd, vd = [], [], [], []
        for W in Ws:
            f, d_, _, _ = prepared(W[E : 2 * E], dt)
            kf.append(f); kd.append(d_)
            f, d_, _, _ = prepared(W[2 * E :], dt)
            vf.append(f); vd.append(d_)
        bk = torch.cat([b.detach()[E : 2 * E] for b in bs])
        bv = torch.cat([b.detach()[2 * E :] for b in bs])
        wk = torch.cat(kf, dim=0)
        K_all = ops.linear_ex(mem, wk, bk, a2=pos, w_shared=True) if pos is not None else ops.linear_fwd(mem, wk, bk)
        V_all = ops.linear_fwd(mem, torch.cat(vf, dim=0), bv)
        shared.wk_d, shared.wv_d = torch.cat(kd, dim=1), torch.cat(vd, dim=1)
        ctx.shared = shared
        ctx.set_materialize_grads(False)
        return K_all, V_all

    @staticmethod
    def backward(ctx, gK, gV):
        sh = ctx.shared
        assert gK is None and gV is None, "the consumers of CrossKVFn hand their gradients over through the shared buffers"
        if sh.dK is None:
            return (None,) * (3 + 2 * sh.n_layers)
        for l in range(sh.n_layers):
            if l not in sh.written:
                sh.dK[:, l * sh.E : (l + 1) * sh.E].zero_()
                sh.dV[:, l * sh.E : (l + 1) * sh.E].zero_()
        d_mem = d_pos = None
        need_pos = sh.pos is not None and ctx.needs_input_grad[1]
        if ctx.needs_input_grad[0] or need_pos:
            d_k = ops.linear_fwd(sh.dK, sh.wk_d)
# ... 59 lines not shown
        sh.written.add(layer)
        dq2 = dq.view(B * Lq, E)
        _wgrad(dq2, q_in, defer, want_bias=True, out=dW_in[:E], dbias=db_in[:E], x2=q_pos)
        _wgrad(dK_all[:, cols], sh.mem, defer, want_bias=True, out=dW_in[E : 2 * E], dbias=db_in[E : 2 * E], x2=sh.pos)
        _wgrad(dV_all[:, cols], sh.mem, defer, want_bias=True, out=dW_in[2 * E :], dbias=db_in[2 * E :])
        need_pos = q_pos is not None and ctx.needs_input_grad[1]
        d_q_in = ops.linear_fwd(dq2, wq_d) if (ctx.needs_input_grad[0] or need_pos) else None
        return (d_q_in if ctx.needs_input_grad[0] else None, d_q_in if need_pos else None, None, None, dW_in, db_in, dW_out, db_out) + (None,) * 12


class _CrossQ1Shared:

    def __init__(self, mem, pos, want_dmem=True):
        self.mem, self.pos = mem, pos
        self.dmem = None
        self.want_dmem = want_dmem
        self.n_layers = 0
        self.coef = None
        self.deferred = {}


class CrossMemFn(Function):

    @staticmethod
    def forward(ctx, mem, shared):
        ctx.shared = shared
        ctx.set_materialize_grads(False)
        return mem.new_empty(0)

    @staticmethod
    def backward(ctx, g):
        sh = ctx.shared
        assert g is None, "the consumers of CrossMemFn hand their gradient over through the shared buffer"
        if sh.coef is not None:
            assert sh.dmem is None
            E = sh.mem.shape[1]
            F_, H = next(iter(sh.deferred.values()))[0].shape[0], next(iter(sh.deferred.values()))[0].shape[1] // E
            for l in range(sh.n_layers):
                if l not in sh.deferred:
                    sh.coef[:, 16 * l : 16 * l + 16].zero_()
            d = ops.cross_q1_dmem(sh.coef, [sh.deferred.get(l) for l in range(sh.n_layers)], F_, sh.mem.shape[0] // F_, H, E)
            sh.coef, sh.deferred = None, {}
            return d, None
        if sh.dmem is None:
            return None, None
        d = sh.dmem if sh.mem.dtype == torch.float32 else ops.cast(sh.dmem, sh.mem.dtype)
        sh.dmem = None
        return d, None


class CrossQ1Fn(Function):

    @staticmethod
    def forward(ctx, q_in, q_pos, token, W_in, b_in, W_out, b_out, key_pad, shared, F, S, H, need_w, p_attn, seed_attn, p_out, seed_out):
        _note_use(ctx.needs_input_grad[3], W_in, b_in, W_out, b_out)
        E = q_in.shape[1]
        dt = q_in.dtype
        scale = 1.0 / math.sqrt(E // H)
        wq_f, wq_d, _, _ = prepared(W_in[:E], dt)
        bq = b_in.detach()[:E]
        q = ops.linear_ex(q_in, wq_f, bq, a2=q_pos, w_shared=True) if q_pos is not None else ops.linear_fwd(q_in, wq_f, bq)
        Wd, bd = W_in.detach(), b_in.detach()
        wk_n, wk_t = ops.head_blocks_expand(Wd[E : 2 * E], None, scale, H, dt)
        wv_n, wv_t = ops.head_blocks_expand(Wd[2 * E :], bd[2 * E :], 1.0, H, dt)
        u = ops.linear_fwd(q, wk_t)
        probs, wavg, zext = ops.cross_q1_fwd(u, shared.mem, shared.pos, key_pad, F, S, H, need_wavg=need_w, dropout_p=p_attn, seed=seed_attn)
        ctxv = ops.linear_fwd(zext, wv_n)
        wo_f, wo_d, _, _ = prepared(W_out, dt)
        out = ops.linear_fwd(ctxv, wo_f, b_out.detach(), dropout_p=p_out, seed=seed_out)
        ctx.save_for_backward(q_in, q_pos, q, u, probs, zext, ctxv, wq_d, wo_d, wk_n, wv_t)
        ctx.cfg = (F, S, H, E, scale, p_attn, seed_attn, p_out, seed_out)
        ctx.params = (W_in, b_in, W_out, b_out)
        ctx.shared = shared
        ctx.layer = shared.n_layers
        shared.n_layers += 1
        return out, (wavg if need_w else None)

    @staticmethod
    def backward(ctx, dout, dwavg):
        _arm()
        q_in, q_pos, q, u, probs, zext, ctxv, wq_d, wo_d, wk_n, wv_t = ctx.saved_tensors
        F, S, H, E, scale, p_attn, seed_attn, p_out, seed_out = ctx.cfg
        sh = ctx.shared
        dt, dev = q_in.dtype, q_in.device
        defer = _can_defer(*ctx.params)
        g = ops.dropout(dout.contiguous(), p_out, seed_out) if p_out > 0 else dout.contiguous()
        dW_in = torch.empty((3 * E, E), dtype=torch.float32, device=dev)
        db_in = torch.empty(3 * E, dtype=torch.float32, device=dev)
        dW_out, db_out = _wgrad(g, ctxv, defer, want_bias=True)
        dctx = ops.linear_fwd(g, wo_d)
        d_zext = ops.linear_fwd(dctx, wv_t)
        Gv = ops.linear_wgrad(dctx, zext)
        ops.head_blocks_extract(Gv, 1.0, dW_in[2 * E :], db_in[2 * E :], H)
        dwa = dwavg.contiguous().float() if dwavg is not None else None
        if sh.want_dmem and dt == torch.bfloat16 and _CROSS_DMEM_DEFER and sh.n_layers <= 8 and sh.dmem is None:
            if sh.coef is None:
                width = (16 * sh.n_layers + 31) // 32 * 32
                sh.coef = torch.empty((F * S, width), dtype=dt, device=dev)
                if width > 16 * sh.n_layers:
                    sh.coef[:, 16 * sh.n_layers :].zero_()
            d_u = ops.cross_q1_bwd_coef(u, sh.mem, sh.pos, probs, d_zext, dwa, sh.coef, 16 * ctx.layer, F, S, H, dropout_p=p_attn, seed=seed_attn)
            sh.deferred[ctx.layer] = (u, d_zext)
        else:
            first = sh.dmem is None
            if not sh.want_dmem:
                dmem = None
            elif first:
                dmem = sh.dmem = torch.empty((F * S, E), dtype=torch.float32, device=dev)
            else:
                dmem = sh.dmem
            d_u = ops.cross_q1_bwd(u, sh.mem, sh.pos, probs, d_zext, dwa, dmem, sh.want_dmem and not first, F, S, H, dropout_p=p_attn, seed=seed_attn)
        dq = ops.linear_fwd(d_u, wk_n)
        Gk = ops.linear_wgrad(q, d_u)
        ops.head_blocks_extract(Gk, scale, dW_in[E : 2 * E], None, H)
        db_in[E : 2 * E].zero_()
        if defer:
            _wgrad(dq, q_in, True, want_bias=True, out=dW_in[:E], dbias=db_in[:E], x2=q_pos)
        else:
            dW_in[:E].zero_()
            db_in[:E].zero_()
            _wgrad(dq, q_in, False, want_bias=True, out=dW_in[:E], dbias=db_in[:E], x2=q_pos)
        need_pos = q_pos is not None and ctx.needs_input_grad[1]
        d_q_in = ops.linear_fwd(dq, wq_d) if (ctx.needs_input_grad[0] or need_pos) else None
        return (d_q_in if ctx.needs_input_grad[0] else None, d_q_in if need_pos else None, None, dW_in, db_in, dW_out, db_out) + (None,) * 10


_CROSS_DMEM_DEFER = _os.environ.get("TD_CROSS_DMEM_DEFER", "1") != "0"


def cross_q1_memory(mem, pos):
    shared = _CrossQ1Shared(mem.detach(), None if pos is None else pos.detach(), want_dmem=mem.requires_grad and torch.is_grad_enabled())
    return CrossMemFn.apply(mem, shared), shared


def multihead_attention_q1(q_in, anchor, W_in, b_in, W_out, b_out, key_pad, F, S, H, need_weights=True, attn_dropout=0.0, out_dropout=0.0,
                           training=False, q_pos=None):
    pa = attn_dropout if training else 0.0
    po = out_dropout if training else 0.0
    token, shared = anchor
    return CrossQ1Fn.apply(q_in, q_pos, token, W_in, b_in, W_out, b_out, key_pad, shared, F, S, H, need_weights,
                           pa, _seed() if pa > 0 else 0, po, _seed() if po > 0 else 0)


def cross_kv(mem, pos, attn_modules):
    E = attn_modules[0].embed_dim
    shared = _CrossKVShared(mem, pos, len(attn_modules), E)
    flat = []
    for m in attn_modules:
        flat += [m.in_proj_weight, m.in_proj_bias]
    K_all, V_all = CrossKVFn.apply(mem, pos, shared, *flat)
    return K_all, V_all, shared


def multihead_attention_prekv(q_in, kv, layer, W_in, b_in, W_out, b_out, key_pad, B, Lq, Lk, H, need_weights=False, attn_dropout=0.0,
                              out_dropout=0.0, training=False, q_pos=None):
    pa = attn_dropout if training else 0.0
    po = out_dropout if training else 0.0
    K_all, V_all, shared = kv
    return MHAPreKVFn.apply(q_in, q_pos, K_all, V_all, W_in, b_in, W_out, b_out, key_pad, shared, layer, B, Lq, Lk, H, need_weights,
                            pa, _seed() if pa > 0 else 0, po, _seed() if po > 0 else 0)


class ReplicaMaps:

    def __init__(self, owner, n: int, hw: int, L: int, device):
        owner = owner.cpu().long()
        F, S = owner.numel(), hw + L
        i32 = lambda t_: t_.to(torch.int32).contiguous().to(device)
        p, l_ = torch.arange(hw), torch.arange(L)
        f = torch.arange(F)
        self.F, self.n, self.hw, self.L, self.S = F, n, hw, L, S
        self.vis_src = i32((owner[:, None] * S + p[None, :]).reshape(-1))
        self.vis_dst = i32((f[:, None] * S + p[None, :]).reshape(-1))
        self.txt_src = i32((owner[:, None] * S + hw + l_[None, :]).reshape(-1))
        self.txt_dst = i32((f[:, None] * S + hw + l_[None, :]).reshape(-1))
        self.all_src = i32((owner[:, None] * S + torch.arange(S)[None, :]).reshape(-1))
        c = torch.arange(n)
        self.iota_vis = i32(torch.arange(n * hw))
        self.clip_vis = i32((c[:, None] * S + p[None, :]).reshape(-1))
        self.clip_txt = i32((c[:, None] * S + hw + l_[None, :]).reshape(-1))
        order = torch.argsort(owner, stable=True)
        counts = torch.bincount(owner, minlength=n)
        starts = torch.cumsum(counts, 0) - counts

        def csr(cols, row_off):
            m = cols.numel()
            per = counts[:, None].expand(n, m).reshape(-1)
            ptr = torch.zeros(n * m + 1, dtype=torch.long)
            ptr[1:] = torch.cumsum(per, 0)
            idx = torch.empty(int(ptr[-1]), dtype=torch.long)
            for ci in range(n):
                fr = order[starts[ci] : starts[ci] + counts[ci]]
                blk = (fr[None, :] * S + row_off + cols[:, None]).reshape(-1)
                idx[ptr[ci * m] : ptr[ci * m] + blk.numel()] = blk
# ... 37 lines not shown
        return frames

    @staticmethod
    def backward(ctx, g):
        _arm()
        mem, fast_mem, wd = ctx.saved_tensors
        maps = ctx.maps
        g = g.contiguous()
        d, dt, dev = g.shape[1], g.dtype, g.device
        n_vis = maps.F * maps.hw
        g_vis = torch.empty((n_vis, d), dtype=dt, device=dev)
        ops.rows_copy(g, maps.vis_dst, g_vis, None, n_vis)
        d_fast = ops.linear_fwd(g_vis, wd) if ctx.needs_input_grad[1] else None
        mix = torch.empty((n_vis, d), dtype=dt, device=dev)
        ops.rows_copy(mem, maps.vis_src, mix, None, n_vis, add=fast_mem)
        dW, db = _wgrad(g_vis, mix, _can_defer(*ctx.params), want_bias=True)
        d_mem = None
        if ctx.needs_input_grad[0]:
            d_mem = torch.empty_like(mem)
            ops.rows_segment_sum(g, maps.seg_txt[0], maps.seg_txt[1], d_mem, maps.clip_txt)
            G = torch.empty((maps.n * maps.hw, d), dtype=dt, device=dev)
            ops.rows_segment_sum(g, maps.seg_vis[0], maps.seg_vis[1], G)
            ops.linear_ex(G, wd, None, residual=G, res_map=maps.iota_vis, out=d_mem, out_map=maps.clip_vis)
        return d_mem, d_fast, dW, db, None


class AttnCoreFn(Function):

    @staticmethod
    def forward(ctx, q, k, v, key_pad, B, Lq, Lk, H, p_drop, seed):
        E = q.shape[1]
        scale = 1.0 / math.sqrt(E // H)
        q3, k3, v3 = q.view(B, Lq, E), k.view(B, Lk, E), v.view(B, Lk, E)
        out, probs, _ = ops.mha_fwd(q3, k3, v3, key_pad, H, scale, need_wavg=False, dropout_p=p_drop, seed=seed)
        ctx.save_for_backward(q3, k3, v3, probs)
        ctx.cfg = (B, Lq, Lk, H, E, scale, p_drop, seed)
        return out.view(B * Lq, E)

    @staticmethod
    def backward(ctx, dout):
        q3, k3, v3, probs = ctx.saved_tensors
        B, Lq, Lk, H, E, scale, p_drop, seed = ctx.cfg
        dq, dk, dv = torch.empty_like(q3), torch.empty_like(k3), torch.empty_like(v3)
        ops.mha_bwd(q3, k3, v3, dout.contiguous().view(B, Lq, E), probs, None, H, scale, dq, dk, dv, dropout_p=p_drop, seed=seed)
        return dq.view(B * Lq, E), dk.view(B * Lk, E), dv.view(B * Lk, E), None, None, None, None, None, None, None


def attention_core(q, k, v, key_pad, B, Lq, Lk, H, dropout_p=0.0, training=False):
    p = dropout_p if training else 0.0
    return AttnCoreFn.apply(q, k, v, key_pad, B, Lq, Lk, H, p, _seed() if p > 0 else 0)


def multihead_attention(q_in, k_in, v_in, W_in, b_in, W_out, b_out, key_pad, B, Lq, Lk, H, need_weights=False,
                        attn_dropout=0.0, out_dropout=0.0, training=False, q_pos=None):
    pa = attn_dropout if training else 0.0
    po = out_dropout if training else 0.0
    return MHAFn.apply(q_in, q_pos, k_in, v_in, W_in, b_in, W_out, b_out, key_pad, B, Lq, Lk, H, need_weights,
                       pa, _seed() if pa > 0 else 0, po, _seed() if po > 0 else 0)


class GeluFn(Function):

    @staticmethod
    def forward(ctx, x):
        x = x.contiguous()
        ctx.save_for_backward(x)
        return ops.gelu_fwd(x)

    @staticmethod
    def backward(ctx, g):
        (x,) = ctx.saved_tensors
        return ops.gelu_bwd(g.contiguous(), x)


def gelu(x):
    return GeluFn.apply(x)


class DropoutFn(Function):
    @staticmethod
    def forward(ctx, x, p, seed):
        ctx.cfg = (p, seed)
        return ops.dropout(x.contiguous(), p, seed)

    @staticmethod
    def backward(ctx, g):
        p, seed = ctx.cfg
        return ops.dropout(g.contiguous(), p, seed), None, None


def dropout(x, p, training):
    if not training or p <= 0:
        return x
    return DropoutFn.apply(x, p, _seed())


class CastFn(Function):

    @staticmethod
    def forward(ctx, x, dtype):
        ctx.src = x.dtype
        return ops.cast(x.contiguous(), dtype)

    @staticmethod
    def backward(ctx, g):
        return ops.cast(g.contiguous(), ctx.src), None


def cast(x, dtype):
    return x if x.dtype == dtype else CastFn.apply(x, dtype)
```

tubedetr_amd/models/transformer.py:

```python
from __future__ import annotations

import copy
import math
import os
from typing import List, Optional

import torch
from torch import Tensor, nn

from .. import functional as Fk
from .. import ops as _ops
from ..util.misc import LRUCache
from .position_encoding import TimeEmbeddingLearned, TimeEmbeddingSine

FAST_MODES_IN_HIP = ("",)
FAST_MODES = ("", "gating", "transformer", "pool", "noslow")


class MultiheadAttention(nn.Module):

    def __init__(self, embed_dim: int, num_heads: int, dropout: float = 0.0):
        super().__init__()
        self.embed_dim, self.num_heads, self.dropout = embed_dim, num_heads, dropout
        self.in_proj_weight = nn.Parameter(torch.empty(3 * embed_dim, embed_dim))
        self.in_proj_bias = nn.Parameter(torch.zeros(3 * embed_dim))
        self.out_proj = nn.Linear(embed_dim, embed_dim)
        nn.init.xavier_uniform_(self.in_proj_weight)
        nn.init.constant_(self.out_proj.bias, 0.0)

    def run_prekv(self, q_in, kv, layer, key_pad, B, Lq, Lk, need_weights, out_dropout, training, q_pos=None):
        return Fk.multihead_attention_prekv(q_in, kv, layer, self.in_proj_weight, self.in_proj_bias, self.out_proj.weight, self.out_proj.bias, key_pad,
                                            B, Lq, Lk, self.num_heads, need_weights, attn_dropout=self.dropout, out_dropout=out_dropout, training=training,
                                            q_pos=q_pos)

    def run_q1(self, q_in, anchor, key_pad, F, S, need_weights, out_dropout, training, q_pos=None):
        return Fk.multihead_attention_q1(q_in, anchor, self.in_proj_weight, self.in_proj_bias, self.out_proj.weight, self.out_proj.bias, key_pad,
                                         F, S, self.num_heads, need_weights, attn_dropout=self.dropout, out_dropout=out_dropout, training=training,
                                         q_pos=q_pos)

    def run(self, q_in, k_in, v_in, key_pad, B, Lq, Lk, need_weights, out_dropout, training, q_pos=None):
        return Fk.multihead_attention(q_in, k_in, v_in, self.in_proj_weight, self.in_proj_bias, self.out_proj.weight,
                                      self.out_proj.bias, key_pad, B, Lq, Lk, self.num_heads, need_weights,
                                      attn_dropout=self.dropout, out_dropout=out_dropout, training=training, q_pos=q_pos)


class TransformerEncoderLayer(nn.Module):
    def __init__(self, d_model, nhead, dim_feedforward=2048, dropout=0.1, activation="relu"):
        super().__init__()
        if activation != "relu":
            raise NotImplementedError("only the reference default activation (relu) is fused in the HIP FFN")
        self.self_attn = MultiheadAttention(d_model, nhead, dropout=dropout)
        self.linear1 = nn.Linear(d_model, dim_feedforward)
        self.linear2 = nn.Linear(dim_feedforward, d_model)
        self.norm1 = nn.LayerNorm(d_model)
        self.norm2 = nn.LayerNorm(d_model)
        self.p = dropout

    def forward(self, src: Tensor, pos: Optional[Tensor], key_pad: Optional[Tensor], B: int, S: int) -> Tensor:
        a, _ = self.self_attn.run(src, None, src, key_pad, B, S, S, False, self.p, self.training, q_pos=pos)
        src = Fk.add_layernorm(a, src, self.norm1.weight, self.norm1.bias, self.norm1.eps)
        f = Fk.ffn(src, self.linear1.weight, self.linear1.bias, self.linear2.weight, self.linear2.bias, self.p, self.training)
        return Fk.add_layernorm(f, src, self.norm2.weight, self.norm2.bias, self.norm2.eps)


class TransformerEncoder(nn.Module):
    def __init__(self, encoder_layer, num_layers, norm=None, return_weights=False):
        super().__init__()
        self.layers = nn.ModuleList([copy.deepcopy(encoder_layer) for _ in range(num_layers)])
        self.num_layers = num_layers
        self.norm = norm
        self.return_weights = return_weights

    def forward(self, src, key_pad, pos, B, S):
        out = src
        for layer in self.layers:
            out = layer(out, pos, key_pad, B, S)
        if self.norm is not None:
            out = Fk.add_layernorm(out, None, self.norm.weight, self.norm.bias, self.norm.eps)
        return out


class TransformerDecoderLayer(nn.Module):
    def __init__(self, d_model, nhead, dim_feedforward=2048, dropout=0.1, activation="relu", no_tsa=False):
        super().__init__()
        if activation != "relu":
            raise NotImplementedError("only relu")
        self.self_attn = MultiheadAttention(d_model, nhead, dropout=dropout)
        self.cross_attn_image = MultiheadAttention(d_model, nhead, dropout=dropout)
        self.linear1 = nn.Linear(d_model, dim_feedforward)
        self.linear2 = nn.Linear(dim_feedforward, d_model)
        self.norm1 = nn.LayerNorm(d_model)
        self.norm3 = nn.LayerNorm(d_model)
        self.norm4 = nn.LayerNorm(d_model)
        self.p = dropout
        self.no_tsa = no_tsa

    def forward(self, tgt, query_pos, mem, pos, query_mask, memory_mask, b: int, t: int, S: int, kv=None, index: int = 0):
        if self.no_tsa:
            a, w = self.self_attn.run(tgt, None, tgt, None, b * t, 1, 1, True, self.p, self.training, q_pos=query_pos)
        else:
            a, w = self.self_attn.run(tgt, None, tgt, query_mask, b, t, t, True, self.p, self.training, q_pos=query_pos)
        tgt = Fk.add_layernorm(a, tgt, self.norm1.weight, self.norm1.bias, self.norm1.eps)
        if isinstance(kv, tuple) and len(kv) == 2:
            a, cw = self.cross_attn_image.run_q1(tgt, kv, memory_mask, b * t, S, True, self.p, self.training, q_pos=query_pos)
        elif kv is not None:
            a, cw = self.cross_attn_image.run_prekv(tgt, kv, index, memory_mask, b * t, 1, S, True, self.p, self.training, q_pos=query_pos)
        else:
            mem_k = Fk.AddFn.apply(mem, pos) if pos is not None else mem
            a, cw = self.cross_attn_image.run(tgt, mem_k, mem, memory_mask, b * t, 1, S, True, self.p, self.training, q_pos=query_pos)
        tgt = Fk.add_layernorm(a, tgt, self.norm3.weight, self.norm3.bias, self.norm3.eps)
        f = Fk.ffn(tgt, self.linear1.weight, self.linear1.bias, self.linear2.weight, self.linear2.bias, self.p, self.training)
        tgt = Fk.add_layernorm(f, tgt, self.norm4.weight, self.norm4.bias, self.norm4.eps)
        return tgt, w, cw


class TransformerDecoder(nn.Module):
    def __init__(self, decoder_layer, num_layers, norm=None, return_intermediate=False, return_weights=False):
        super().__init__()
        self.layers = nn.ModuleList([copy.deepcopy(decoder_layer) for _ in range(num_layers)])
        self.num_layers = num_layers
        self.norm = norm
        self.return_intermediate = return_intermediate
        self.return_weights = return_weights

    def forward(self, tgt, query_pos, mem, pos, query_mask, memory_mask, b, t, S):
        inter, ws, cws = [], [], []
        out = tgt
        att = self.layers[0].cross_attn_image
        if (os.environ.get("TD_CROSS_Q1", "1") != "0" and att.embed_dim == 256 and att.num_heads == 8 and S <= 320
                and not (pos is not None and pos.requires_grad)):
            kv = Fk.cross_q1_memory(mem, pos)
        else:
            kv = Fk.cross_kv(mem, pos, [l.cross_attn_image for l in self.layers]) if os.environ.get("TD_KV_HOIST", "1") != "0" else None
        for i, layer in enumerate(self.layers):
            out, w, cw = layer(out, query_pos, mem, pos, query_mask, memory_mask, b, t, S, kv=kv, index=i)
            if self.return_intermediate:
                inter.append(Fk.add_layernorm(out, None, self.norm.weight, self.norm.bias, self.norm.eps))
                ws.append(w)
                cws.append(cw)
        if not self.return_intermediate:
            out = Fk.add_layernorm(out, None, self.norm.weight, self.norm.bias, self.norm.eps) if self.norm is not None else out
            return (out, w, cw) if self.return_weights else out
        hs = torch.stack(inter)
        if not self.return_weights:
            return hs
        return hs, torch.stack(ws), torch.stack(cws)


class FeatureResizer(nn.Module):

    def __init__(self, input_feat_size, output_feat_size, dropout, do_ln=True):
        super().__init__()
        self.do_ln = do_ln
        self.fc = nn.Linear(input_feat_size, output_feat_size, bias=True)
        self.layer_norm = nn.LayerNorm(output_feat_size, eps=1e-12)
        self.p = dropout

    def forward(self, rows: Tensor) -> Tensor:
        x = Fk.linear(rows, self.fc.weight, self.fc.bias)
        if self.do_ln:
            x = Fk.add_layernorm(x, None, self.layer_norm.weight, self.layer_norm.bias, self.layer_norm.eps)
        return Fk.dropout(x, self.p, self.training)

# ... 324 lines not shown
```

tubedetr_amd/ops.py:

```python
from __future__ import annotations

import os

import ctypes as C
from typing import Optional, Tuple

import torch

from . import _hip
from ._hip import ConvDesc, Epilogue, check, dtype_code, ptr, stream_ptr

Tensor = torch.Tensor


class _ZeroArena:

    def __init__(self, chunk: int):
        self.chunk = chunk
        self.buf = None
        self.off = 0

    def take(self, shape, device) -> torch.Tensor:
        n = 1
        for d_ in shape:
# ... 19 lines not shown


def zeros_f32(shape, device) -> torch.Tensor:
    if not _USE_ARENA:
        return torch.zeros(shape, dtype=torch.float32, device=device)
    shape = tuple(shape) if not isinstance(shape, int) else (shape,)
    if device.type == "cuda" and torch.cuda.is_current_stream_capturing():
        sp = stream_ptr()
        if sp not in _CAPTURE_ARENAS:
            _CAPTURE_ARENAS[sp] = _ZeroArena(256 * 1024)
        return _CAPTURE_ARENAS[sp].take(shape, device)
    if _CAPTURE_ARENAS:
        _CAPTURE_ARENAS.clear()
    key = (str(device), stream_ptr() if device.type == "cuda" else 0)
    arena = _ARENAS.get(key)
    if arena is None:
        arena = _ARENAS[key] = _ZeroArena(32 * 1024 * 1024)
    return arena.take(shape, device)


def vec_of(dt: torch.dtype) -> int:
    return 8 if dt == torch.bfloat16 else 4


def pad_to(n: int, m: int) -> int:
    return (n + m - 1) // m * m


def conv_out(h: int, k: int, stride: int, pad: int) -> int:
    return (h + 2 * pad - k) // stride + 1


def _desc(N, Hs, Ws, Cs, Ho, Wo, R, S, stride, pad, mode, Nc, ldc, out_sp=1, out_H=0, out_W=0, stride_w=None, pad_w=None) -> ConvDesc:
    if stride_w is None and pad_w is None:
        return ConvDesc(N, Hs, Ws, Cs, Ho, Wo, R, S, stride, pad, mode, Nc, ldc, out_sp, out_H, out_W)
    return ConvDesc(N, Hs, Ws, Cs, Ho, Wo, R, S, stride, pad, mode, Nc, ldc, out_sp, out_H, out_W, 1, stride if stride_w is None else stride_w,
                    pad if pad_w is None else pad_w)


_DROPOUT_COUNTER = [None]


def set_dropout_counter(counter: Optional[torch.Tensor]) -> None:
    if counter is not None:
        assert counter.is_cuda and counter.numel() == 1 and counter.element_size() == 4
    _DROPOUT_COUNTER[0] = counter


def _ctr():
    c = _DROPOUT_COUNTER[0]
    return c.data_ptr() if c is not None else None


def _epi(bias=None, residual=None, mask_src=None, relu=False, sigmoid=False, dropout_p=0.0, seed=0, alpha=1.0) -> Epilogue:
    return Epilogue(ptr(bias), ptr(residual), ptr(mask_src), int(relu), int(sigmoid), float(dropout_p), int(seed) & 0xFFFFFFFF, float(alpha),
                    _ctr() if dropout_p > 0 else None)


def conv_gemm_raw(src: Tensor, w: Tensor, out: Tensor, desc: ConvDesc, epi: Optional[Epilogue]):
    check(_hip.lib().td_conv_gemm(ptr(src), ptr(w), ptr(out), C.byref(desc), C.byref(epi) if epi is not None else None,
                                  dtype_code(src.dtype), stream_ptr()), "td_conv_gemm")


def conv_fwd(x: Tensor, w_fwd: Tensor, bias: Optional[Tensor], R: int, S: int, stride: int, pad: int, *,
             residual: Optional[Tensor] = None, relu: bool = False, out: Optional[Tensor] = None) -> Tensor:
    N, H, W, Cs = x.shape
    Co = w_fwd.shape[0]
    assert w_fwd.shape[1] == R * S * Cs and w_fwd.dtype == x.dtype and x.is_contiguous() and w_fwd.is_contiguous()
    Ho, Wo = conv_out(H, R, stride, pad), conv_out(W, S, stride, pad)
    y = out if out is not None else torch.empty((N, Ho, Wo, Co), dtype=x.dtype, device=x.device)
    conv_gemm_raw(x, w_fwd, y, _desc(N, H, W, Cs, Ho, Wo, R, S, stride, pad, 0, Co, Co), _epi(bias, residual, None, relu))
    return y


def conv_dgrad(g: Tensor, w_dgrad: Tensor, in_hw: Tuple[int, int], R: int, S: int, stride: int, pad: int, *,
               residual: Optional[Tensor] = None, mask_src: Optional[Tensor] = None, out: Optional[Tensor] = None) -> Tensor:
    N, Hg, Wg, Co = g.shape
    H, W = in_hw
    Ci = w_dgrad.shape[0]
    assert w_dgrad.shape[1] == R * S * Co and g.is_contiguous()
    dx = out if out is not None else torch.empty((N, H, W, Ci), dtype=g.dtype, device=g.device)
    conv_gemm_raw(g, w_dgrad, dx, _desc(N, Hg, Wg, Co, H, W, R, S, stride, pad, 1, Ci, Ci), _epi(None, residual, mask_src))
    return dx


def conv1x1s_dgrad_scatter(g: Tensor, w_dgrad: Tensor, dx: Tensor, stride: int, *, mask_src: Optional[Tensor] = None):
    N, Hg, Wg, Co = g.shape
    _, H, W, Ci = dx.shape
    d = _desc(N, Hg, Wg, Co, Hg, Wg, 1, 1, 1, 0, 0, Ci, Ci, stride, H, W)
    conv_gemm_raw(g, w_dgrad, dx, d, _epi(None, dx, mask_src))
    return dx


def conv_wgrad(g: Tensor, x: Tensor, R: int, S: int, stride: int, pad: int, *, out: Optional[Tensor] = None, splits: int = 0) -> Tensor:
    N, H, W, Cs = x.shape
    _, Ho, Wo, Co = g.shape
    dw = out if out is not None else zeros_f32((Co, R * S * Cs), x.device)
    d = _desc(N, H, W, Cs, Ho, Wo, R, S, stride, pad, 0, Co, Co)
    check(_hip.lib().td_conv_wgrad(ptr(g), ptr(x), ptr(dw), C.byref(d), Co, dtype_code(x.dtype), splits, stream_ptr()), "td_conv_wgrad")
    return dw


class _JobTables:

    RING = 12

    def __init__(self):
        self.slots, self.retired, self.cap, self.next = [], [], 0, 0

# ... 33 lines not shown


def conv_wgrad_batch(jobs) -> list:
    jobs = list(jobs)
    arr = (_hip.WgradJob * len(jobs))()
    outs = []
    for a, (g, x, R, S, stride, pad, scale, ci_real) in zip(arr, jobs):
        N, H, W, Cs = x.shape
        _, Ho, Wo, Co = g.shape
        assert g.is_contiguous() and x.is_contiguous() and g.dtype == x.dtype
        dw = torch.empty((Co, ci_real, R, S), dtype=torch.float32, device=x.device)
        outs.append(dw)
        a.g, a.src, a.dW, a.scale = g.data_ptr(), x.data_ptr(), dw.data_ptr(), (scale.data_ptr() if scale is not None else None)
        a.d = _desc(N, H, W, Cs, Ho, Wo, R, S, stride, pad, 0, Co, Co)
        a.ldg, a.ci_real, a.dbias = Co, ci_real, None
    nbytes = _hip.lib().td_conv_wgrad_batch_table_bytes(len(jobs))
    th, td_, done = job_tables.take(nbytes, jobs[0][0].device)
    check(_hip.lib().td_conv_wgrad_batch(arr, len(jobs), dtype_code(jobs[0][0].dtype), th.data_ptr(), td_.data_ptr(), nbytes, stream_ptr()),
          "td_conv_wgrad_batch")
    done()
    return outs


def linear_wgrad_batch(jobs) -> None:
    if not jobs:
        return
    key0 = (jobs[0][0].dtype, jobs[0][0].device)
    if any((j[0].dtype, j[0].device) != key0 for j in jobs):
        groups: dict = {}
        for j in jobs:
            groups.setdefault((j[0].dtype, j[0].device), []).append(j)
        for sub in groups.values():
            linear_wgrad_batch(sub)
        return
    arr = (_hip.WgradJob * len(jobs))()
    for a, job in zip(arr, jobs):
        g, x, dw_ptr, db_ptr = job[:4]
        M, K = x.shape
        Nn = g.shape[1]
        assert g.shape[0] == M and g.stride(1) == 1 and x.is_contiguous() and g.dtype == x.dtype
        a.g, a.src, a.dW, a.scale, a.dbias = g.data_ptr(), x.data_ptr(), dw_ptr, None, db_ptr
        a.d = _desc(1, M, 1, K, M, 1, 1, 1, 1, 0, 0, Nn, Nn)
        a.ldg, a.ci_real = g.stride(0), K
        a.accumulate = int(len(job) > 4 and bool(job[4]))
    nbytes = _hip.lib().td_conv_wgrad_batch_table_bytes(len(jobs))
    dev = jobs[0][0].device
    th, td_, done = job_tables.take(nbytes, dev)
    check(_hip.lib().td_conv_wgrad_batch(arr, len(jobs), dtype_code(jobs[0][0].dtype), th.data_ptr(), td_.data_ptr(), nbytes, stream_ptr()),
          "td_conv_wgrad_batch(linears)")
    done()


def linear_fwd(x: Tensor, w: Tensor, bias: Optional[Tensor] = None, *, residual=None, relu=False, sigmoid=False,
               mask_src=None, dropout_p=0.0, seed=0, alpha=1.0, out: Optional[Tensor] = None) -> Tensor:
    M, K = x.shape
    Nn = w.shape[0]
    assert w.shape[1] == K and w.dtype == x.dtype and x.is_contiguous() and w.is_contiguous()
    y = out if out is not None else torch.empty((M, Nn), dtype=x.dtype, device=x.device)
    conv_gemm_raw(x, w, y, _desc(1, M, 1, K, M, 1, 1, 1, 1, 0, 0, Nn, Nn), _epi(bias, residual, mask_src, relu, sigmoid, dropout_p, seed, alpha))
    return y


def pw_chain2(y2: Tensor, w3: Tensor, b3: Tensor, residual: Tensor, w1: Tensor, b1: Tensor, *, out: Optional[Tensor] = None,
              h1: Optional[Tensor] = None) -> Tuple[Tensor, Tensor]:
    M, P = y2.shape
    assert y2.dtype == torch.bfloat16 and w3.shape == (4 * P, P) and w1.shape == (P, 4 * P) and residual.shape == (M, 4 * P)
    assert y2.is_contiguous() and w3.is_contiguous() and w1.is_contiguous() and residual.is_contiguous()
    assert b3.dtype == torch.float32 and b1.dtype == torch.float32 and b3.numel() == 4 * P and b1.numel() == P
    out = out if out is not None else torch.empty((M, 4 * P), dtype=y2.dtype, device=y2.device)
    h1 = h1 if h1 is not None else torch.empty((M, P), dtype=y2.dtype, device=y2.device)
    check(_hip.lib().td_pw_chain2(ptr(y2), ptr(w3), ptr(b3), ptr(residual), ptr(out), ptr(w1), ptr(b1), ptr(h1), M, P, dtype_code(y2.dtype),
                                  stream_ptr()), "td_pw_chain2")
    return out, h1


def _rows2d(t: Tensor):
    assert t.dim() == 2 and t.stride(1) == 1, "row-major 2-D operand expected (unit column stride)"
    return t


def linear_ex(a1: Tensor, w: Tensor, bias: Optional[Tensor] = None, *, a2: Optional[Tensor] = None, a1_map: Optional[Tensor] = None,
              a2_map: Optional[Tensor] = None, w_shared: bool = False, out: Optional[Tensor] = None, out_map: Optional[Tensor] = None,
              out_rows: Optional[int] = None, residual: Optional[Tensor] = None, res_map: Optional[Tensor] = None, relu=False, mask_src=None,
              dropout_p=0.0, seed=0, alpha=1.0) -> Tensor:
    _rows2d(a1)
    K1 = a1.shape[1]
    K2 = _rows2d(a2).shape[1] if a2 is not None else 0
    M = int(a1_map.numel()) if a1_map is not None else a1.shape[0]
    Nn = w.shape[0]
    assert w.is_contiguous() and w.dtype == a1.dtype and w.shape[1] == (K1 if (w_shared or a2 is None) else K1 + K2)
    for m_ in (a1_map, a2_map, out_map, res_map):
        assert m_ is None or (m_.dtype == torch.int32 and m_.is_contiguous() and m_.numel() == M)
    if out is None:
        out = torch.empty((out_rows if out_rows is not None else M, Nn), dtype=a1.dtype, device=a1.device)
    _rows2d(out)
    x = _hip.LinearExDesc()
    x.M, x.N, x.K1, x.K2 = M, Nn, K1, K2
    x.lda1, x.lda2, x.ldc = a1.stride(0), (a2.stride(0) if a2 is not None else 0), out.stride(0)
    x.ldr = _rows2d(residual).stride(0) if residual is not None else 0
    x.w_shared = int(bool(w_shared and a2 is not None))
    x.rows1, x.rows2 = a1.shape[0], (a2.shape[0] if a2 is not None else 0)
    x.a1_map, x.a2_map, x.out_map, x.res_map = ptr(a1_map), ptr(a2_map), ptr(out_map), ptr(res_map)
    epi = _epi(bias, residual, mask_src, relu, False, dropout_p, seed, alpha)
    check(_hip.lib().td_linear_ex(ptr(a1), ptr(a2), ptr(w), ptr(out), C.byref(x), C.byref(epi), dtype_code(a1.dtype), stream_ptr()), "td_linear_ex")
    return out


def rows_copy(src: Tensor, src_map: Optional[Tensor], dst: Tensor, dst_map: Optional[Tensor], n_rows: int, add: Optional[Tensor] = None) -> Tensor:
    _rows2d(src), _rows2d(dst)
    cols = src.shape[1]
    assert dst.shape[1] == cols and dst.dtype == src.dtype and (add is None or (_rows2d(add).shape[1] == cols and add.dtype == src.dtype and add.shape[0] >= n_rows))
    for m_ in (src_map, dst_map):
# ... 52 lines not shown


def nchw_to_nhwc(x: Tensor, dtype: torch.dtype, cpad: int) -> Tensor:
    N, Cc, H, W = x.shape
    assert x.dtype == torch.float32 and x.is_contiguous()
    y = torch.empty((N, H, W, cpad), dtype=dtype, device=x.device)
    check(_hip.lib().td_nchw_to_nhwc(ptr(x), ptr(y), N, Cc, H, W, cpad, dtype_code(dtype), stream_ptr()), "td_nchw_to_nhwc")
    return y


def nhwc_to_nchw(x: Tensor) -> Tensor:
    N, H, W, Cc = x.shape
    y = torch.empty((N, Cc, H, W), dtype=torch.float32, device=x.device)
    check(_hip.lib().td_nhwc_to_nchw(ptr(x), ptr(y), N, Cc, H, W, dtype_code(x.dtype), stream_ptr()), "td_nhwc_to_nchw")
    return y


def cast(x: Tensor, dtype: torch.dtype) -> Tensor:
    if x.dtype == dtype:
        return x
    y = torch.empty(x.shape, dtype=dtype, device=x.device)
    check(_hip.lib().td_cast(ptr(x.contiguous()), ptr(y), x.numel(), dtype_code(x.dtype), dtype_code(dtype), stream_ptr()), "td_cast")
    return y


def maxpool3x3s2(x: Tensor) -> Tensor:
    N, H, W, Cc = x.shape
    y = torch.empty((N, conv_out(H, 3, 2, 1), conv_out(W, 3, 2, 1), Cc), dtype=x.dtype, device=x.device)
    check(_hip.lib().td_maxpool3x3s2(ptr(x), ptr(y), N, H, W, Cc, dtype_code(x.dtype), stream_ptr()), "td_maxpool3x3s2")
    return y


def add_layernorm_fwd(x: Tensor, r: Optional[Tensor], gamma: Tensor, beta: Tensor, eps: float, save: bool = True):
    rows, cols = x.shape
    y = torch.empty_like(x)
    s = torch.empty_like(x) if (save and r is not None) else None
    mean = torch.empty(rows, dtype=torch.float32, device=x.device) if save else None
    rstd = torch.empty(rows, dtype=torch.float32, device=x.device) if save else None
    check(_hip.lib().td_add_layernorm_fwd(ptr(x), ptr(r), ptr(gamma), ptr(beta), ptr(y), ptr(s), ptr(mean), ptr(rstd), rows, cols, eps,
                                          dtype_code(x.dtype), stream_ptr()), "td_add_layernorm_fwd")
    return y, (s if r is not None else x), mean, rstd


def add_layernorm_bwd(dy: Tensor, s: Tensor, mean: Tensor, rstd: Tensor, gamma: Tensor, extra: Optional[Tensor] = None):
    rows, cols = dy.shape
    ds = torch.empty_like(dy)
    dgamma = zeros_f32(cols, dy.device)
    dbeta = zeros_f32(cols, dy.device)
    check(_hip.lib().td_add_layernorm_bwd(ptr(dy), ptr(s), ptr(mean), ptr(rstd), ptr(gamma), ptr(extra), ptr(ds), ptr(dgamma), ptr(dbeta),
                                          rows, cols, dtype_code(dy.dtype), stream_ptr()), "td_add_layernorm_bwd")
    return ds, dgamma, dbeta


def colsum(g: Tensor, out: Optional[Tensor] = None) -> Tensor:
    rows, cols = g.shape
    o = out if out is not None else zeros_f32(cols, g.device)
    check(_hip.lib().td_colsum(ptr(g), ptr(o), rows, cols, cols, dtype_code(g.dtype), stream_ptr()), "td_colsum")
    return o


def add(a: Tensor, b: Optional[Tensor]) -> Tensor:
    y = torch.empty_like(a)
    check(_hip.lib().td_add(ptr(a), ptr(b), ptr(y), a.numel(), dtype_code(a.dtype), stream_ptr()), "td_add")
    return y


def relu_bwd(dy: Tensor, y: Tensor, scale: float = 1.0) -> Tensor:
    g = torch.empty_like(dy)
    check(_hip.lib().td_relu_bwd(ptr(dy), ptr(y), ptr(g), dy.numel(), scale, dtype_code(dy.dtype), stream_ptr()), "td_relu_bwd")
    return g


def pos_sine(mask: Tensor, npf: int, dtype: torch.dtype, temperature: float = 10000.0, rows: Optional[int] = None) -> Tensor:
    N, h, w = mask.shape
    m8 = mask.to(torch.uint8).contiguous()
    rows = h * w if rows is None else int(rows)
    pos = torch.empty((N, rows, 2 * npf), dtype=dtype, device=mask.device)
    check(_hip.lib().td_pos_sine(ptr(m8), ptr(pos), N, h, w, npf, temperature, rows, dtype_code(dtype), stream_ptr()), "td_pos_sine")
    return pos


def mha_fwd(q: Tensor, k: Tensor, v: Tensor, key_pad: Optional[Tensor], H: int, scale: float, *, need_wavg: bool = False,
            dropout_p: float = 0.0, seed: int = 0):
    B, Lq, E = q.shape
    Lk = k.shape[1]
    hd = E // H
    for t_ in (q, k, v):
        assert t_.stride(2) == 1 and t_.stride(0) == t_.shape[1] * t_.stride(1)
    out = torch.empty((B, Lq, E), dtype=q.dtype, device=q.device)
    probs = torch.empty((B, H, Lq, Lk), dtype=torch.float32, device=q.device)
    wavg = torch.empty((B, Lq, Lk), dtype=torch.float32, device=q.device) if need_wavg else None
    kp = key_pad.to(torch.uint8).contiguous() if key_pad is not None else None
    check(_hip.lib().td_mha_fwd(ptr(q), ptr(k), ptr(v), ptr(kp), ptr(out), ptr(probs), ptr(wavg), B, H, Lq, Lk, hd, q.stride(1), k.stride(1),
                                v.stride(1), E, scale, dropout_p, seed & 0xFFFFFFFF, _ctr() if dropout_p > 0 else None, dtype_code(q.dtype), stream_ptr()),
          "td_mha_fwd")
    return out, probs, wavg


def mha_lean_ok(q: Tensor, k: Tensor, v: Tensor, H: int) -> bool:
    if os.environ.get("TD_MHA_LEAN", "1") == "0":
        return False
    E = q.shape[2]
    return (q.dtype == torch.bfloat16 and E // H == 32
            and all(t_.stride(1) % 8 == 0 and t_.data_ptr() % 16 == 0 for t_ in (q, k, v)))


# ... 133 lines not shown
```

Baseline: 106.0.

## Fuse add-LayerNorm into attention and FFN autograd functions with fused backward dropout

Moves the post-sublayer residual add + LayerNorm inside the MHA and FFN autograd functions, on by default through TD_FUSED_TAIL. In backward, a new LN-backward kernel also writes the dropout-masked gradient, which removes the separate dropout kernel. The residual gradient add is folded into the dgrad GEMM epilogue, with bf16 rounding of the GEMM result to match the previous numerics. This cuts kernel launches and extra passes over activations in the transformer layers, at the cost of more complex autograd plumbing and one extra gradient buffer.

```diff
diff --git a/include/tubedetr_hip.h b/include/tubedetr_hip.h
--- a/include/tubedetr_hip.h
+++ b/include/tubedetr_hip.h
@@ -63,6 +63,7 @@
   uint32_t dropout_seed;
   float alpha;
   const uint32_t* dropout_counter;
+  int residual_rounded;
 } td_epilogue;
 
 int td_conv_gemm(const void* src, const void* wmat, void* out, const td_conv_desc* d, const td_epilogue* e,
@@ -157,6 +158,9 @@
 int td_add_layernorm_bwd(const void* dy, const void* s, const float* mean, const float* rstd, const float* gamma,
                          const void* extra, void* ds, float* dgamma, float* dbeta, int rows, int cols, int dtype,
                          td_stream_t stream);
+int td_add_layernorm_bwd_drop(const void* dy, const void* s, const float* mean, const float* rstd, const float* gamma,
+                              const void* extra, void* ds, void* ds_drop, float* dgamma, float* dbeta, int rows, int cols,
+                              float dropout_p, uint32_t dropout_seed, const uint32_t* dropout_counter, int dtype, td_stream_t stream);
 
 int td_colsum(const void* g, float* out, int rows, int cols, int ld, int dtype, td_stream_t stream);
 int td_add(const void* a, const void* b, void* y, size_t n, int dtype, td_stream_t stream);
diff --git a/tubedetr_amd/_hip.py b/tubedetr_amd/_hip.py
--- a/tubedetr_amd/_hip.py
+++ b/tubedetr_amd/_hip.py
@@ -6,7 +6,7 @@
 import torch
 
 TD_F32, TD_BF16 = 0, 1
-EXPECTED_ABI = 10
+EXPECTED_ABI = 11
 _LIB_PATH = os.environ.get("TD_HIP_LIB") or os.path.join(os.path.dirname(os.path.abspath(__file__)), "lib", "libtubedetr_hip.so")
 _lib = None
 
@@ -52,6 +52,7 @@
         ("dropout_seed", C.c_uint32),
         ("alpha", C.c_float),
         ("dropout_counter", C.c_void_p),
+        ("residual_rounded", C.c_int),
     ]
 
 
@@ -86,6 +87,7 @@
     "td_maxpool3x3s2": [_P, _P, _I, _I, _I, _I, _I, _P],
     "td_add_layernorm_fwd": [_P, _P, _P, _P, _P, _P, _P, _P, _I, _I, _F, _I, _P],
     "td_add_layernorm_bwd": [_P, _P, _P, _P, _P, _P, _P, _P, _P, _I, _I, _I, _P],
+    "td_add_layernorm_bwd_drop": [_P, _P, _P, _P, _P, _P, _P, _P, _P, _P, _I, _I, _F, _U32, _P, _I, _P],
     "td_colsum": [_P, _P, _I, _I, _I, _I, _P],
     "td_add": [_P, _P, _P, _SZ, _I, _P],
     "td_relu_bwd": [_P, _P, _P, _SZ, _F, _I, _P],
diff --git a/tubedetr_amd/csrc/api.cpp b/tubedetr_amd/csrc/api.cpp
--- a/tubedetr_amd/csrc/api.cpp
+++ b/tubedetr_amd/csrc/api.cpp
@@ -125,4 +125,4 @@
 }
 
 extern "C" const char* td_last_error(void) { return td::g_err; }
-extern "C" int td_abi_version(void) { return 10; }
+extern "C" int td_abi_version(void) { return 11; }
diff --git a/tubedetr_amd/csrc/elementwise.hip b/tubedetr_amd/csrc/elementwise.hip
--- a/tubedetr_amd/csrc/elementwise.hip
+++ b/tubedetr_amd/csrc/elementwise.hip
@@ -145,12 +145,19 @@
   }
 }
 
-template <int NJ>
+struct LnDrop {
+  void* out;
+  float scale;
+  uint32_t thresh, seed;
+  const uint32_t* seed_dev;
+};
+template <int NJ, bool DROP = false>
 __global__ __launch_bounds__(256) void add_layernorm_bwd_v4_kernel(const u16* __restrict__ dy, const u16* __restrict__ s, const float* __restrict__ mean,
                                                                    const float* __restrict__ rstd, const float* __restrict__ gamma,
                                                                    const u16* __restrict__ extra, u16* __restrict__ ds, float* dgamma, float* dbeta,
-                                                                   int rows) {
+                                                                   int rows, LnDrop dr = LnDrop{}) {
   constexpr int cols = NJ * 256;
+  const uint32_t drop_seed = DROP ? effective_seed(dr.seed, dr.thresh ? dr.seed_dev : nullptr) : 0u;
   const int lane = threadIdx.x & 63;
   const int wid = blockIdx.x * 4 + (threadIdx.x >> 6);
   const int nw = gridDim.x * 4;
@@ -195,7 +202,15 @@
 #pragma unroll
         for (int e = 0; e < 4; ++e) o[e] += ex[e];
       }
-      *(uint2*)(ds + base + 256 * j) = pack4_bf16(o);
+      const uint2 pk = pack4_bf16(o);
+      *(uint2*)(ds + base + 256 * j) = pk;
+      if constexpr (DROP) {
+        float q[4];
+        unpack4v(pk, q);
+#pragma unroll
+        for (int e = 0; e < 4; ++e) q[e] = dropout_keep(drop_seed, (uint32_t)(base + 256 * j + e), dr.thresh) ? q[e] * dr.scale : 0.f;
+        *(uint2*)((u16*)dr.out + base + 256 * j) = pack4_bf16(q);
+      }
     }
   }
   __shared__ float redg[4][cols], redb[4][cols];
@@ -217,7 +232,8 @@
 template <typename T>
 __global__ __launch_bounds__(256) void add_layernorm_bwd_kernel(const T* dy, const T* s, const float* mean, const float* rstd,
                                                                 const float* gamma, const T* extra, T* ds, float* dgamma,
-                                                                float* dbeta, int rows, int cols) {
+                                                                float* dbeta, int rows, int cols, LnDrop dr = LnDrop{}) {
+  const uint32_t drop_seed = dr.out ? effective_seed(dr.seed, dr.thresh ? dr.seed_dev : nullptr) : 0u;
   const int lane = threadIdx.x & 63;
   const int wid = blockIdx.x * 4 + (threadIdx.x >> 6);
   const int nw = gridDim.x * 4;
@@ -253,6 +269,10 @@
         float o = rs * (dg[j] - c1 - xh[j] * c2);
         if (extra) o += Elem<T>::load(extra, base + c);
         Elem<T>::store(ds, base + c, o);
+        if (dr.out) {
+          const float q = Elem<T>::load(ds, base + c);
+          Elem<T>::store(dr.out, base + c, dropout_keep(drop_seed, (uint32_t)(base + c), dr.thresh) ? q * dr.scale : 0.f);
+        }
       }
     }
   }
@@ -551,6 +571,40 @@
   return check_launch("td_add_layernorm_bwd");
 }
 
+extern "C" int td_add_layernorm_bwd_drop(const void* dy, const void* s, const float* mean, const float* rstd, const float* gamma,
+                                         const void* extra, void* ds, void* ds_drop, float* dgamma, float* dbeta, int rows, int cols,
+                                         float dropout_p, uint32_t dropout_seed, const uint32_t* dropout_counter, int dtype, td_stream_t stream) {
+  TD_REQUIRE(dy && s && mean && rstd && gamma && ds && ds_drop, "td_add_layernorm_bwd_drop: null pointer");
+  TD_REQUIRE(cols <= 64 * LN_MAXJ, "td_add_layernorm_bwd_drop: cols > %d", 64 * LN_MAXJ);
+  TD_REQUIRE(dropout_p >= 0.f && dropout_p < 1.f, "td_add_layernorm_bwd_drop: dropout_p out of range");
+  TD_REQUIRE((double)rows * cols < 4294967296.0, "td_add_layernorm_bwd_drop: 2^32 elements or more");
+  if (rows == 0) return TD_OK;
+  LnDrop dr;
+  dr.out = ds_drop;
+  dr.thresh = dropout_p > 0.f ? (uint32_t)((double)dropout_p * 4294967296.0) : 0u;
+  if (dropout_p > 0.f && !dr.thresh) dr.thresh = 1;
+  dr.scale = 1.f / (1.f - dropout_p);
+  dr.seed = dropout_seed;
+  dr.seed_dev = dropout_counter;
+  hipStream_t st = (hipStream_t)stream;
+  unsigned g = (rows + 3) / 4;
+  if (dtype == TD_BF16 && (cols == 256 || cols == 768) && aligned8(dy, s, ds, extra) && ((uintptr_t)ds_drop & 7) == 0) {
+    unsigned gv = (rows + 31) / 32;
+    if (gv > 1024) gv = 1024;
+    if (deterministic()) gv = 1;
+    if (cols == 256) add_layernorm_bwd_v4_kernel<1, true><<<gv, 256, 0, st>>>((const u16*)dy, (const u16*)s, mean, rstd, gamma, (const u16*)extra, (u16*)ds, dgamma, dbeta, rows, dr);
+    else add_layernorm_bwd_v4_kernel<3, true><<<gv, 256, 0, st>>>((const u16*)dy, (const u16*)s, mean, rstd, gamma, (const u16*)extra, (u16*)ds, dgamma, dbeta, rows, dr);
+    return check_launch("td_add_layernorm_bwd_drop");
+  }
+  if (g > 256) g = 256;
+  if (deterministic()) g = 1;
+  TD_DISPATCH(dtype,
+              (add_layernorm_bwd_kernel<u16><<<g, 256, 0, st>>>((const u16*)dy, (const u16*)s, mean, rstd, gamma, (const u16*)extra, (u16*)ds, dgamma, dbeta, rows, cols, dr)),
+              (add_layernorm_bwd_kernel<float><<<g, 256, 0, st>>>((const float*)dy, (const float*)s, mean, rstd, gamma, (const float*)extra, (float*)ds, dgamma, dbeta, rows, cols, dr)),
+              "td_add_layernorm_bwd_drop");
+  return check_launch("td_add_layernorm_bwd_drop");
+}
+
 extern "C" int td_colsum(const void* g, float* out, int rows, int cols, int ld, int dtype, td_stream_t stream) {
   TD_REQUIRE(g && out, "td_colsum: null pointer");
   if (rows == 0 || cols == 0) return TD_OK;
diff --git a/tubedetr_amd/csrc/gemm_conv.hip b/tubedetr_amd/csrc/gemm_conv.hip
--- a/tubedetr_amd/csrc/gemm_conv.hip
+++ b/tubedetr_amd/csrc/gemm_conv.hip
@@ -26,6 +26,7 @@
   const char* residual;
   const char* mask_src;
   int relu, sigmoid;
+  int res_round;
   float alpha;
   uint32_t drop_thresh;
   float drop_scale;
@@ -92,6 +93,7 @@
   bf16x2_t v = {(__bf16)lo, (__bf16)hi};
   return *(uint32_t*)&v;
 }
+__device__ __forceinline__ float bf16_rn(float x) { return __uint_as_float(pack_bf16x2(x, 0.f) << 16); }
 template <typename T>
 __device__ __forceinline__ void unpack16(const uint4& v, float (&o)[16 / sizeof(T)]);
 template <>
@@ -470,6 +472,10 @@
       if (p.residual) {
         float r8[EPL];
         unpack16<T>(res[it], r8);
+        if (sizeof(T) == 2 && p.res_round) {
+#pragma unroll
+          for (int r = 0; r < EPL; ++r) v[r] = bf16_rn(v[r]);
+        }
 #pragma unroll
         for (int r = 0; r < EPL; ++r) v[r] += r8[r];
       }
@@ -496,7 +502,7 @@
       const int cnt = min(EPL, d.Nc - n);
       for (int r = 0; r < cnt; ++r) {
         float x = v[r];
-        if (p.residual) x += Elem<T>::load(p.residual, (GX ? roffs[it] : off) + r);
+        if (p.residual) x = ((sizeof(T) == 2 && p.res_round) ? bf16_rn(x) : x) + Elem<T>::load(p.residual, (GX ? roffs[it] : off) + r);
         if (p.relu) x = fmaxf(x, 0.f);
         if (p.sigmoid) x = sigmoidf_(x);
         if (p.mask_src) x = Elem<T>::load(p.mask_src, off + r) > 0.f ? x : 0.f;
@@ -804,6 +810,10 @@
           const int m = m0 + wy * WM + j * 16 + lr;
           if (m < p.M) {
             const uint2 rr = *(const uint2*)(p.residual + ((size_t)m * d.ldc + n0 + wx * WN + i * 16 + lg * 4) * ES);
+            if (p.res_round) {
+#pragma unroll
+              for (int r = 0; r < 4; ++r) v[r] = bf16_rn(v[r]);
+            }
             v[0] += __uint_as_float(rr.x << 16); v[1] += __uint_as_float(rr.x & 0xffff0000u);
             v[2] += __uint_as_float(rr.y << 16); v[3] += __uint_as_float(rr.y & 0xffff0000u);
           }
@@ -1101,6 +1111,10 @@
       if (p.residual) {
         float r8[EPL];
         unpack16<T>(res[b][it], r8);
+        if (p.res_round) {
+#pragma unroll
+          for (int r = 0; r < EPL; ++r) v[r] = bf16_rn(v[r]);
+        }
 #pragma unroll
         for (int r = 0; r < EPL; ++r) v[r] += r8[r];
       }
@@ -1268,6 +1282,10 @@
         if constexpr (RES) {
           float r8[EPL];
           unpack16<T>(make_uint4(res[RB][it].x, res[RB][it].y, res[RB][it].z, res[RB][it].w), r8);
+          if (p.res_round) {
+#pragma unroll
+            for (int r = 0; r < EPL; ++r) v[r] = bf16_rn(v[r]);
+          }
 #pragma unroll
           for (int r = 0; r < EPL; ++r) v[r] += r8[r];
         }
@@ -2174,6 +2192,7 @@
   if (e) {
     p.bias = e->bias;
     p.residual = (const char*)e->residual;
+    p.res_round = e->residual && e->residual_rounded && dtype == TD_BF16;
     p.mask_src = (const char*)e->mask_src;
     p.relu = e->relu;
     p.sigmoid = e->sigmoid;
@@ -2361,6 +2380,7 @@
   if (e) {
     p.bias = e->bias;
     p.residual = (const char*)e->residual;
+    p.res_round = e->residual && e->residual_rounded && dtype == TD_BF16;
     p.mask_src = (const char*)e->mask_src;
     p.relu = e->relu;
     p.sigmoid = e->sigmoid;
diff --git a/tubedetr_amd/functional.py b/tubedetr_amd/functional.py
--- a/tubedetr_amd/functional.py
+++ b/tubedetr_amd/functional.py
@@ -235,6 +235,19 @@
     return dW, db
 
 
+def fused_tail() -> bool:
+    return _os.environ.get("TD_FUSED_TAIL", "1") != "0"
+
+
+def _ln_bwd_head(dy, ln_saved, p, seed):
+    sres, mean, rstd, gamma = ln_saved
+    dy = dy if dy.is_contiguous() else dy.contiguous()
+    if p > 0:
+        return ops.add_layernorm_bwd_drop(dy, sres, mean, rstd, gamma, p, seed)
+    ds, dg, db = ops.add_layernorm_bwd(dy, sres, mean, rstd, gamma)
+    return ds, ds, dg, db
+
+
 class LinearFn(Function):
 
     @staticmethod
@@ -289,13 +302,18 @@
 class FFNFn(Function):
 
     @staticmethod
-    def forward(ctx, x, W1, b1, W2, b2, p: float, seed1: int, seed2: int):
+    def forward(ctx, x, W1, b1, W2, b2, p: float, seed1: int, seed2: int, ln_g=None, ln_b=None, ln_eps: float = 0.0):
         _note_use(ctx.needs_input_grad[1], W1, b1, W2, b2)
         w1f, w1d, _, _ = prepared(W1, x.dtype)
         w2f, w2d, _, _ = prepared(W2, x.dtype)
         h = ops.linear_fwd(x, w1f, b1.detach(), relu=True, dropout_p=p, seed=seed1)
         y = ops.linear_fwd(h, w2f, b2.detach(), dropout_p=p, seed=seed2)
-        ctx.save_for_backward(x, h, w1d, w2d)
+        ctx.ln = ln_g is not None
+        if ctx.ln:
+            y, sres, mean, rstd = ops.add_layernorm_fwd(y, x, ln_g.detach(), ln_b.detach(), ln_eps)
+            ctx.save_for_backward(x, h, w1d, w2d, sres, mean, rstd, ln_g.detach())
+        else:
+            ctx.save_for_backward(x, h, w1d, w2d)
         ctx.cfg = (p, seed1, seed2)
         ctx.params = (W1, b1, W2, b2)
         return y
@@ -303,20 +321,24 @@
     @staticmethod
     def backward(ctx, dy):
         _arm()
-        x, h, w1d, w2d = ctx.saved_tensors
+        x, h, w1d, w2d, *ln_saved = ctx.saved_tensors
         p, seed1, seed2 = ctx.cfg
         defer = _can_defer(*ctx.params)
-        g2 = ops.dropout(dy.contiguous(), p, seed2) if p > 0 else dy.contiguous()
+        ds = dgam = dbet = None
+        if ctx.ln:
+            ds, g2, dgam, dbet = _ln_bwd_head(dy, ln_saved, p, seed2)
+        else:
+            g2 = ops.dropout(dy.contiguous(), p, seed2) if p > 0 else dy.contiguous()
         dW2, db2 = _wgrad(g2, h, defer, want_bias=True)
         dh = ops.linear_fwd(g2, w2d, mask_src=h, alpha=1.0 / (1.0 - p) if p > 0 else 1.0)
         dW1, db1 = _wgrad(dh, x, defer, want_bias=True)
-        dx = ops.linear_fwd(dh, w1d) if ctx.needs_input_grad[0] else None
-        return dx, dW1, db1, dW2, db2, None, None, None
-
-
-def ffn(x, W1, b1, W2, b2, dropout_p=0.0, training=False):
+        dx = ops.linear_fwd(dh, w1d, residual=ds, residual_rounded=ds is not None) if ctx.needs_input_grad[0] else None
+        return dx, dW1, db1, dW2, db2, None, None, None, dgam, dbet, None
+
+
+def ffn(x, W1, b1, W2, b2, dropout_p=0.0, training=False, ln=None):
     p = dropout_p if training else 0.0
-    return FFNFn.apply(x, W1, b1, W2, b2, p, _seed() if p > 0 else 0, _seed() if p > 0 else 0)
+    return FFNFn.apply(x, W1, b1, W2, b2, p, _seed() if p > 0 else 0, _seed() if p > 0 else 0, *(ln if ln is not None else ()))
 
 
 class AddLayerNormFn(Function):
@@ -353,7 +375,8 @@
 class MHAFn(Function):
 
     @staticmethod
-    def forward(ctx, q_in, q_pos, k_in, v_in, W_in, b_in, W_out, b_out, key_pad, B, Lq, Lk, H, need_w, p_attn, seed_attn, p_out, seed_out):
+    def forward(ctx, q_in, q_pos, k_in, v_in, W_in, b_in, W_out, b_out, key_pad, B, Lq, Lk, H, need_w, p_attn, seed_attn, p_out, seed_out,
+                ln_g=None, ln_b=None, ln_eps: float = 0.0):
         _note_use(ctx.needs_input_grad[4], W_in, b_in, W_out, b_out)
         E = q_in.shape[1]
         dt = q_in.dtype
@@ -386,7 +409,13 @@
             kp = None
         wo_f, wo_d, _, _ = prepared(W_out, dt)
         out = ops.linear_fwd(ctxv.view(B * Lq, E), wo_f, b_out.detach(), dropout_p=p_out, seed=seed_out)
-        ctx.save_for_backward(q_in, q_pos, k_in, v_in, q, k, v, probs, ctxv, wv_d, wo_d, *wd_list)
+        ctx.ln = ln_g is not None
+        ln_saved = ()
+        if ctx.ln:
+            assert same_qk and v_in.shape == q_in.shape
+            out, sres, mean, rstd = ops.add_layernorm_fwd(out, q_in, ln_g.detach(), ln_b.detach(), ln_eps)
+            ln_saved = (sres, mean, rstd, ln_g.detach())
+        ctx.save_for_backward(q_in, q_pos, k_in, v_in, q, k, v, probs, ctxv, wv_d, wo_d, *wd_list, *ln_saved)
         ctx.lean, ctx.kp = lean, kp
         ctx.cfg = (B, Lq, Lk, H, E, same_qk, scale, p_attn, seed_attn, p_out, seed_out)
         ctx.params = (W_in, b_in, W_out, b_out)
@@ -400,7 +429,12 @@
         dt = q_in.dtype
         dev = q_in.device
         defer = _can_defer(*ctx.params)
-        g = ops.dropout(dout.contiguous(), p_out, seed_out) if p_out > 0 else dout.contiguous()
+        ds = dgam = dbet = None
+        if ctx.ln:
+            wd_list, ln_saved = wd_list[:-4], wd_list[-4:]
+            ds, g, dgam, dbet = _ln_bwd_head(dout, ln_saved, p_out, seed_out)
+        else:
+            g = ops.dropout(dout.contiguous(), p_out, seed_out) if p_out > 0 else dout.contiguous()
         if defer:
             dW_in = torch.empty((3 * E, E), dtype=torch.float32, device=dev)
             db_in = torch.empty(3 * E, dtype=torch.float32, device=dev)
@@ -423,6 +457,16 @@
             ops.mha_bwd(q, k, v, dctx, probs, dwa, H, scale, dq, dk, dv, dropout_p=p_attn, seed=seed_attn)
         dv2 = dv.view(B * Lk, E)
         _wgrad(dv2, v_in, defer, want_bias=True, out=dW_in[2 * E :], dbias=db_in[2 * E :])
+        need_pos = q_pos is not None and ctx.needs_input_grad[1]
+        if ctx.ln:
+            dqk2 = dqk.view(B * Lq, 2 * E)
+            _wgrad(dqk2, q_in, defer, want_bias=True, out=dW_in[: 2 * E], dbias=db_in[: 2 * E], x2=q_pos)
+            d_pos = ops.linear_fwd(dqk2, wd_list[0]) if need_pos else None
+            d_x = None
+            if ctx.needs_input_grad[0]:
+                d_x = ops.add(ds, d_pos) if need_pos else ops.linear_fwd(dqk2, wd_list[0], residual=ds, residual_rounded=True)
+                d_x = ops.linear_fwd(dv2, wv_d, residual=d_x, residual_rounded=True)
+            return (d_x, d_pos, None, None, dW_in, db_in, dW_out, db_out) + (None,) * 10 + (dgam, dbet, None)
         d_v_in = ops.linear_fwd(dv2, wv_d) if ctx.needs_input_grad[3] else None
         d_q_in = d_k_in = None
         need_q = ctx.needs_input_grad[0] or (q_pos is not None and ctx.needs_input_grad[1])
@@ -440,7 +484,7 @@
             if ctx.needs_input_grad[2]:
                 d_k_in = ops.linear_fwd(dk2, wd_list[1])
         return (d_q_in if ctx.needs_input_grad[0] else None, d_q_in if (q_pos is not None and ctx.needs_input_grad[1]) else None, d_k_in, d_v_in,
-                dW_in, db_in, dW_out, db_out) + (None,) * 10
+                dW_in, db_in, dW_out, db_out) + (None,) * 10 + (None, None, None)
 
 
 class _CrossKVShared:
@@ -606,7 +650,8 @@
 class CrossQ1Fn(Function):
 
     @staticmethod
-    def forward(ctx, q_in, q_pos, token, W_in, b_in, W_out, b_out, key_pad, shared, F, S, H, need_w, p_attn, seed_attn, p_out, seed_out):
+    def forward(ctx, q_in, q_pos, token, W_in, b_in, W_out, b_out, key_pad, shared, F, S, H, need_w, p_attn, seed_attn, p_out, seed_out,
+                ln_g=None, ln_b=None, ln_eps: float = 0.0):
         _note_use(ctx.needs_input_grad[3], W_in, b_in, W_out, b_out)
         E = q_in.shape[1]
         dt = q_in.dtype
@@ -622,7 +667,12 @@
         ctxv = ops.linear_fwd(zext, wv_n)
         wo_f, wo_d, _, _ = prepared(W_out, dt)
         out = ops.linear_fwd(ctxv, wo_f, b_out.detach(), dropout_p=p_out, seed=seed_out)
-        ctx.save_for_backward(q_in, q_pos, q, u, probs, zext, ctxv, wq_d, wo_d, wk_n, wv_t)
+        ctx.ln = ln_g is not None
+        ln_saved = ()
+        if ctx.ln:
+            out, sres, mean, rstd = ops.add_layernorm_fwd(out, q_in, ln_g.detach(), ln_b.detach(), ln_eps)
+            ln_saved = (sres, mean, rstd, ln_g.detach())
+        ctx.save_for_backward(q_in, q_pos, q, u, probs, zext, ctxv, wq_d, wo_d, wk_n, wv_t, *ln_saved)
         ctx.cfg = (F, S, H, E, scale, p_attn, seed_attn, p_out, seed_out)
         ctx.params = (W_in, b_in, W_out, b_out)
         ctx.shared = shared
@@ -633,12 +683,16 @@
     @staticmethod
     def backward(ctx, dout, dwavg):
         _arm()
-        q_in, q_pos, q, u, probs, zext, ctxv, wq_d, wo_d, wk_n, wv_t = ctx.saved_tensors
+        q_in, q_pos, q, u, probs, zext, ctxv, wq_d, wo_d, wk_n, wv_t, *ln_saved = ctx.saved_tensors
         F, S, H, E, scale, p_attn, seed_attn, p_out, seed_out = ctx.cfg
         sh = ctx.shared
         dt, dev = q_in.dtype, q_in.device
         defer = _can_defer(*ctx.params)
-        g = ops.dropout(dout.contiguous(), p_out, seed_out) if p_out > 0 else dout.contiguous()
+        ds = dgam = dbet = None
+        if ctx.ln:
+            ds, g, dgam, dbet = _ln_bwd_head(dout, ln_saved, p_out, seed_out)
+        else:
+            g = ops.dropout(dout.contiguous(), p_out, seed_out) if p_out > 0 else dout.contiguous()
         dW_in = torch.empty((3 * E, E), dtype=torch.float32, device=dev)
         db_in = torch.empty(3 * E, dtype=torch.float32, device=dev)
         dW_out, db_out = _wgrad(g, ctxv, defer, want_bias=True)
@@ -675,8 +729,14 @@
             db_in[:E].zero_()
             _wgrad(dq, q_in, False, want_bias=True, out=dW_in[:E], dbias=db_in[:E], x2=q_pos)
         need_pos = q_pos is not None and ctx.needs_input_grad[1]
+        if ctx.ln:
+            d_pos = ops.linear_fwd(dq, wq_d) if need_pos else None
+            d_x = None
+            if ctx.needs_input_grad[0]:
+                d_x = ops.add(ds, d_pos) if need_pos else ops.linear_fwd(dq, wq_d, residual=ds, residual_rounded=True)
+            return (d_x, d_pos, None, dW_in, db_in, dW_out, db_out) + (None,) * 10 + (dgam, dbet, None)
         d_q_in = ops.linear_fwd(dq, wq_d) if (ctx.needs_input_grad[0] or need_pos) else None
-        return (d_q_in if ctx.needs_input_grad[0] else None, d_q_in if need_pos else None, None, dW_in, db_in, dW_out, db_out) + (None,) * 10
+        return (d_q_in if ctx.needs_input_grad[0] else None, d_q_in if need_pos else None, None, dW_in, db_in, dW_out, db_out) + (None,) * 10 + (None, None, None)
 
 
 _CROSS_DMEM_DEFER = _os.environ.get("TD_CROSS_DMEM_DEFER", "1") != "0"
@@ -688,12 +748,12 @@
 
 
 def multihead_attention_q1(q_in, anchor, W_in, b_in, W_out, b_out, key_pad, F, S, H, need_weights=True, attn_dropout=0.0, out_dropout=0.0,
-                           training=False, q_pos=None):
+                           training=False, q_pos=None, ln=None):
     pa = attn_dropout if training else 0.0
     po = out_dropout if training else 0.0
     token, shared = anchor
     return CrossQ1Fn.apply(q_in, q_pos, token, W_in, b_in, W_out, b_out, key_pad, shared, F, S, H, need_weights,
-                           pa, _seed() if pa > 0 else 0, po, _seed() if po > 0 else 0)
+                           pa, _seed() if pa > 0 else 0, po, _seed() if po > 0 else 0, *(ln if ln is not None else ()))
 
 
 def cross_kv(mem, pos, attn_modules):
@@ -837,11 +897,12 @@
 
 
 def multihead_attention(q_in, k_in, v_in, W_in, b_in, W_out, b_out, key_pad, B, Lq, Lk, H, need_weights=False,
-                        attn_dropout=0.0, out_dropout=0.0, training=False, q_pos=None):
+                        attn_dropout=0.0, out_dropout=0.0, training=False, q_pos=None, ln=None):
     pa = attn_dropout if training else 0.0
     po = out_dropout if training else 0.0
+    assert ln is None or (k_in is None and v_in is q_in)
     return MHAFn.apply(q_in, q_pos, k_in, v_in, W_in, b_in, W_out, b_out, key_pad, B, Lq, Lk, H, need_weights,
-                       pa, _seed() if pa > 0 else 0, po, _seed() if po > 0 else 0)
+                       pa, _seed() if pa > 0 else 0, po, _seed() if po > 0 else 0, *(ln if ln is not None else ()))
 
 
 class GeluFn(Function):
diff --git a/tubedetr_amd/models/transformer.py b/tubedetr_amd/models/transformer.py
--- a/tubedetr_amd/models/transformer.py
+++ b/tubedetr_amd/models/transformer.py
@@ -33,15 +33,19 @@
                                             B, Lq, Lk, self.num_heads, need_weights, attn_dropout=self.dropout, out_dropout=out_dropout, training=training,
                                             q_pos=q_pos)
 
-    def run_q1(self, q_in, anchor, key_pad, F, S, need_weights, out_dropout, training, q_pos=None):
+    def run_q1(self, q_in, anchor, key_pad, F, S, need_weights, out_dropout, training, q_pos=None, ln=None):
         return Fk.multihead_attention_q1(q_in, anchor, self.in_proj_weight, self.in_proj_bias, self.out_proj.weight, self.out_proj.bias, key_pad,
                                          F, S, self.num_heads, need_weights, attn_dropout=self.dropout, out_dropout=out_dropout, training=training,
-                                         q_pos=q_pos)
-
-    def run(self, q_in, k_in, v_in, key_pad, B, Lq, Lk, need_weights, out_dropout, training, q_pos=None):
+                                         q_pos=q_pos, ln=ln)
+
+    def run(self, q_in, k_in, v_in, key_pad, B, Lq, Lk, need_weights, out_dropout, training, q_pos=None, ln=None):
         return Fk.multihead_attention(q_in, k_in, v_in, self.in_proj_weight, self.in_proj_bias, self.out_proj.weight,
                                       self.out_proj.bias, key_pad, B, Lq, Lk, self.num_heads, need_weights,
-                                      attn_dropout=self.dropout, out_dropout=out_dropout, training=training, q_pos=q_pos)
+                                      attn_dropout=self.dropout, out_dropout=out_dropout, training=training, q_pos=q_pos, ln=ln)
+
+
+def _ln(norm: nn.LayerNorm):
+    return (norm.weight, norm.bias, norm.eps)
 
 
 class TransformerEncoderLayer(nn.Module):
@@ -57,6 +61,9 @@
         self.p = dropout
 
     def forward(self, src: Tensor, pos: Optional[Tensor], key_pad: Optional[Tensor], B: int, S: int) -> Tensor:
+        if Fk.fused_tail():
+            src, _ = self.self_attn.run(src, None, src, key_pad, B, S, S, False, self.p, self.training, q_pos=pos, ln=_ln(self.norm1))
+            return Fk.ffn(src, self.linear1.weight, self.linear1.bias, self.linear2.weight, self.linear2.bias, self.p, self.training, ln=_ln(self.norm2))
         a, _ = self.self_attn.run(src, None, src, key_pad, B, S, S, False, self.p, self.training, q_pos=pos)
         src = Fk.add_layernorm(a, src, self.norm1.weight, self.norm1.bias, self.norm1.eps)
         f = Fk.ffn(src, self.linear1.weight, self.linear1.bias, self.linear2.weight, self.linear2.bias, self.p, self.training)
@@ -96,12 +103,17 @@
         self.no_tsa = no_tsa
 
     def forward(self, tgt, query_pos, mem, pos, query_mask, memory_mask, b: int, t: int, S: int, kv=None, index: int = 0):
+        fused = Fk.fused_tail()
+        ln1 = _ln(self.norm1) if fused else None
         if self.no_tsa:
-            a, w = self.self_attn.run(tgt, None, tgt, None, b * t, 1, 1, True, self.p, self.training, q_pos=query_pos)
-        else:
-            a, w = self.self_attn.run(tgt, None, tgt, query_mask, b, t, t, True, self.p, self.training, q_pos=query_pos)
-        tgt = Fk.add_layernorm(a, tgt, self.norm1.weight, self.norm1.bias, self.norm1.eps)
+            a, w = self.self_attn.run(tgt, None, tgt, None, b * t, 1, 1, True, self.p, self.training, q_pos=query_pos, ln=ln1)
+        else:
+            a, w = self.self_attn.run(tgt, None, tgt, query_mask, b, t, t, True, self.p, self.training, q_pos=query_pos, ln=ln1)
+        tgt = a if fused else Fk.add_layernorm(a, tgt, self.norm1.weight, self.norm1.bias, self.norm1.eps)
         if isinstance(kv, tuple) and len(kv) == 2:
+            if fused:
+                tgt, cw = self.cross_attn_image.run_q1(tgt, kv, memory_mask, b * t, S, True, self.p, self.training, q_pos=query_pos, ln=_ln(self.norm3))
+                return Fk.ffn(tgt, self.linear1.weight, self.linear1.bias, self.linear2.weight, self.linear2.bias, self.p, self.training, ln=_ln(self.norm4)), w, cw
             a, cw = self.cross_attn_image.run_q1(tgt, kv, memory_mask, b * t, S, True, self.p, self.training, q_pos=query_pos)
         elif kv is not None:
             a, cw = self.cross_attn_image.run_prekv(tgt, kv, index, memory_mask, b * t, 1, S, True, self.p, self.training, q_pos=query_pos)
@@ -109,6 +121,8 @@
             mem_k = Fk.AddFn.apply(mem, pos) if pos is not None else mem
             a, cw = self.cross_attn_image.run(tgt, mem_k, mem, memory_mask, b * t, 1, S, True, self.p, self.training, q_pos=query_pos)
         tgt = Fk.add_layernorm(a, tgt, self.norm3.weight, self.norm3.bias, self.norm3.eps)
+        if fused:
+            return Fk.ffn(tgt, self.linear1.weight, self.linear1.bias, self.linear2.weight, self.linear2.bias, self.p, self.training, ln=_ln(self.norm4)), w, cw
         f = Fk.ffn(tgt, self.linear1.weight, self.linear1.bias, self.linear2.weight, self.linear2.bias, self.p, self.training)
         tgt = Fk.add_layernorm(f, tgt, self.norm4.weight, self.norm4.bias, self.norm4.eps)
         return tgt, w, cw
diff --git a/tubedetr_amd/ops.py b/tubedetr_amd/ops.py
--- a/tubedetr_amd/ops.py
+++ b/tubedetr_amd/ops.py
@@ -95,9 +95,9 @@
     return c.data_ptr() if c is not None else None
 
 
-def _epi(bias=None, residual=None, mask_src=None, relu=False, sigmoid=False, dropout_p=0.0, seed=0, alpha=1.0) -> Epilogue:
+def _epi(bias=None, residual=None, mask_src=None, relu=False, sigmoid=False, dropout_p=0.0, seed=0, alpha=1.0, residual_rounded=False) -> Epilogue:
     return Epilogue(ptr(bias), ptr(residual), ptr(mask_src), int(relu), int(sigmoid), float(dropout_p), int(seed) & 0xFFFFFFFF, float(alpha),
-                    _ctr() if dropout_p > 0 else None)
+                    _ctr() if dropout_p > 0 else None, int(residual_rounded))
 
 
 def conv_gemm_raw(src: Tensor, w: Tensor, out: Tensor, desc: ConvDesc, epi: Optional[Epilogue]):
@@ -237,12 +237,12 @@
 
 
 def linear_fwd(x: Tensor, w: Tensor, bias: Optional[Tensor] = None, *, residual=None, relu=False, sigmoid=False,
-               mask_src=None, dropout_p=0.0, seed=0, alpha=1.0, out: Optional[Tensor] = None) -> Tensor:
+               mask_src=None, dropout_p=0.0, seed=0, alpha=1.0, out: Optional[Tensor] = None, residual_rounded: bool = False) -> Tensor:
     M, K = x.shape
     Nn = w.shape[0]
     assert w.shape[1] == K and w.dtype == x.dtype and x.is_contiguous() and w.is_contiguous()
     y = out if out is not None else torch.empty((M, Nn), dtype=x.dtype, device=x.device)
-    conv_gemm_raw(x, w, y, _desc(1, M, 1, K, M, 1, 1, 1, 1, 0, 0, Nn, Nn), _epi(bias, residual, mask_src, relu, sigmoid, dropout_p, seed, alpha))
+    conv_gemm_raw(x, w, y, _desc(1, M, 1, K, M, 1, 1, 1, 1, 0, 0, Nn, Nn), _epi(bias, residual, mask_src, relu, sigmoid, dropout_p, seed, alpha, residual_rounded))
     return y
 
 
@@ -401,6 +401,18 @@
     return ds, dgamma, dbeta
 
 
+def add_layernorm_bwd_drop(dy: Tensor, s: Tensor, mean: Tensor, rstd: Tensor, gamma: Tensor, p: float, seed: int, extra: Optional[Tensor] = None):
+    rows, cols = dy.shape
+    ds = torch.empty_like(dy)
+    ds_drop = torch.empty_like(dy)
+    dgamma = zeros_f32(cols, dy.device)
+    dbeta = zeros_f32(cols, dy.device)
+    check(_hip.lib().td_add_layernorm_bwd_drop(ptr(dy), ptr(s), ptr(mean), ptr(rstd), ptr(gamma), ptr(extra), ptr(ds), ptr(ds_drop), ptr(dgamma),
+                                               ptr(dbeta), rows, cols, p, seed & 0xFFFFFFFF, _ctr() if p > 0 else None, dtype_code(dy.dtype),
+                                               stream_ptr()), "td_add_layernorm_bwd_drop")
+    return ds, ds_drop, dgamma, dbeta
+
+
 def colsum(g: Tensor, out: Optional[Tensor] = None) -> Tensor:
     rows, cols = g.shape
     o = out if out is not None else zeros_f32(cols, g.device)
```

Measured after the change: 106.1, median of 6. Within noise of the previous version (+0.2%).
